# jac99/Egonn

Hardware: AMD Instinct MI355X
Metric: LiDAR scans/sec (descriptor extraction), 50k-pt clouds @ 0.1m voxel (higher is better)
Workload: dtype f32

## Files before the change

egonn_amd/_lib.py:

```python
from __future__ import annotations

import ctypes as C
import os
from typing import List, Optional, Sequence

import numpy as np
import torch

_HERE = os.path.dirname(os.path.abspath(__file__))
LIB_PATH = os.path.join(_HERE, "lib", "libegonn_hip.so")

QUANT_CARTESIAN, QUANT_POLAR = 0, 1
FLAG_DISABLE_GLOBAL, FLAG_DISABLE_LOCAL, FLAG_IGNORE_KP_REGRESSOR, FLAG_BF16 = 1, 2, 4, 8
FLAG_POOL_SPOC, FLAG_POOL_MAC = 16, 32
MINKFPN_SPLIT_TOPDOWN = 1
MINKFPN_BLOCKS = {'BasicBlock': 0, 'ECABasicBlock': 1}
MINKFPN_POOLING = {None: 0, 'GeM': 1, 'MAC': 2, 'SPoC': 3}

_P = C.c_void_p
_SIGS = [
    ("egonn_ctx_create", C.c_int, [C.POINTER(_P), C.c_int, C.c_int]),
    ("egonn_ctx_destroy", None, [_P]),
    ("egonn_last_error", C.c_char_p, []),
    ("egonn_debug_set_naive_conv", C.c_int, [_P, C.c_int]),
    ("egonn_debug_set_ksplit", C.c_int, [_P, C.c_int, C.c_int, C.c_int, C.c_int, C.c_int]),
    ("egonn_debug_set_resident", C.c_int, [_P, C.c_int, C.c_int]),
    ("egonn_debug_keep_level_features", C.c_int, [_P, C.c_int]),
    ("egonn_debug_set_trace", C.c_int, [_P]),
    ("egonn_prepare_maps", C.c_int, [_P, C.c_int, _P]),
    ("egonn_debug_rowgroup_tables", C.c_int, [_P, C.c_int, C.c_int, _P, _P, C.c_int64, C.POINTER(C.c_int64), _P]),
    ("egonn_debug_rowgroup_perm", C.c_int, [_P, C.c_int, C.c_int, _P, C.c_int64, C.POINTER(C.c_int64), _P]),
    ("egonn_debug_radix_sort_scratch_bytes", C.c_int64, [C.c_int64, C.c_int]),
    ("egonn_debug_radix_sort", C.c_int, [_P, _P, _P, _P, C.c_int64, C.c_int, _P, _P, C.c_int, C.c_int, C.c_int,
                                         C.POINTER(C.c_int32), _P, C.c_int64, _P]),
    ("egonn_voxelize", C.c_int, [_P, _P, C.POINTER(C.c_int64), C.c_int, C.c_int, C.POINTER(C.c_float), _P]),
    ("egonn_ctx_reserve", C.c_int, [_P, C.c_int64, C.c_int, C.POINTER(C.c_int64)]),
    ("egonn_voxelize_device", C.c_int, [_P, _P, C.c_int64, _P, C.c_int, C.c_int, C.POINTER(C.c_float), _P]),
    ("egonn_plan_status", C.c_int, [_P, _P]),
    ("egonn_ctx_set_exact_fp32", C.c_int, [_P, C.c_int]),
    ("egonn_ctx_set_operand_autoscale", C.c_int, [_P, C.c_int]),
    ("egonn_level_capacity", C.c_int, [_P, C.c_int, C.POINTER(C.c_int64)]),
    ("egonn_graph_begin", C.c_int, [_P]),
    ("egonn_graph_end", C.c_int, [_P, C.POINTER(_P)]),
    ("egonn_graph_launch", C.c_int, [_P, _P]),
    ("egonn_graph_destroy", None, [_P]),
    ("egonn_coords_set", C.c_int, [_P, _P, C.c_int64, C.c_int, _P]),
    ("egonn_level_count", C.c_int, [_P, C.c_int, C.POINTER(C.c_int64)]),
    ("egonn_level_batch_offsets", C.c_int, [_P, C.c_int, C.POINTER(C.c_int64)]),
    ("egonn_level_coords", C.c_int, [_P, C.c_int, _P, _P]),
    ("egonn_input_index", C.c_int, [_P, _P, _P]),
    ("egonn_conv", C.c_int, [_P, C.c_int, C.c_int, C.c_int, _P, C.c_int, _P, C.c_int, _P, _P, C.c_int, _P, _P]),
    ("egonn_conv_transpose", C.c_int, [_P, C.c_int, _P, C.c_int, _P, C.c_int, _P, _P]),
    ("egonn_sparse_conv", C.c_int, [_P, C.c_int, C.c_int, _P, C.c_int, _P, C.c_int, C.c_int, _P, _P, C.c_int, _P, _P, _P]),
    ("egonn_map_groups", C.c_int, [_P, C.c_int, C.c_int, C.POINTER(C.c_int64), C.POINTER(C.c_int64), _P]),
    ("egonn_global_avg_pool", C.c_int, [_P, C.c_int, _P, C.c_int, _P, _P]),
    ("egonn_bn_fold", C.c_int, [_P, _P, _P, _P, C.c_float, C.c_int, _P, _P, _P]),
    ("egonn_block_tail", C.c_int, [_P, C.c_int, _P, _P, C.c_int, _P, C.c_int, _P, _P]),
    ("egonn_gem", C.c_int, [_P, C.c_int, _P, C.c_int, _P, _P, _P]),
    ("egonn_global_max_pool", C.c_int, [_P, C.c_int, _P, C.c_int, _P, _P]),
    ("egonn_netvlad", C.c_int, [_P, C.c_int, _P, C.c_int, _P, _P, _P, _P, _P, _P, _P, _P, _P, _P, C.c_int, C.c_int, _P, _P]),
    ("egonn_netvlad_train_forward", C.c_int, [_P, C.c_int, _P, C.c_int, C.c_int, _P, _P, _P, _P, C.c_float, C.c_float, _P, _P,
                                              _P, C.c_int, _P, _P, _P, _P, _P, _P, _P]),
    ("egonn_netvlad_train_backward", C.c_int, [_P, C.c_int, _P, C.c_int, C.c_int, _P, _P, _P, _P, C.c_int, _P, _P, _P, _P, _P,
                                               _P, _P, _P, _P, _P, _P, _P]),
    ("egonn_global_max_pool_argmax", C.c_int, [_P, C.c_int, _P, C.c_int, _P, _P, _P]),
    ("egonn_global_max_pool_backward", C.c_int, [_P, C.c_int, _P, _P, C.c_int, _P, _P]),
    ("egonn_sigmoid_gate", C.c_int, [_P, _P, _P, C.c_int64, _P, _P, _P, _P]),
    ("egonn_add", C.c_int, [_P, _P, C.c_int64, _P, _P]),
    ("egonn_gather_input", C.c_int, [_P, _P, C.c_int, _P, _P]),
    ("egonn_model_create", C.c_int, [C.POINTER(_P)]),
    ("egonn_model_destroy", None, [_P]),
    ("egonn_model_set_tensor", C.c_int, [_P, C.c_char_p, _P, C.c_int, C.POINTER(C.c_int64)]),
    ("egonn_model_finalize", C.c_int, [_P, _P]),
    ("egonn_forward", C.c_int, [_P, _P, _P, C.c_int, C.POINTER(C.c_float), C.c_int, _P, _P, _P, _P, _P]),
    ("egonn_forward_level_features", C.c_int, [_P, C.c_int, _P, C.c_int, _P]),
    ("egonn_minkfpn_finalize", C.c_int, [_P, C.c_int, C.POINTER(C.c_int), C.POINTER(C.c_int), C.c_int, C.c_int, C.c_int, C.c_int, _P]),
    ("egonn_minkfpn_out_level", C.c_int, [C.c_int, C.c_int, C.POINTER(C.c_int)]),
    ("egonn_minkfpn_forward", C.c_int, [_P, _P, C.c_int, _P, _P, _P]),
    ("egonn_topdown_step", C.c_int, [_P, C.c_int, _P, _P, _P, _P, C.c_int, C.c_int, _P, _P]),
    ("egonn_select_keypoints", C.c_int, [_P, _P, _P, _P, C.c_int, _P, _P, _P, _P, _P]),
    ("egonn_topk_rows", C.c_int, [_P, _P, C.c_int, C.c_int, _P, _P, _P]),
    ("egonn_triplet_loss_scratch_floats", C.c_int64, [C.c_int]),
    ("egonn_triplet_loss", C.c_int, [_P, C.c_int, C.c_int, _P, _P, C.c_float, _P, _P, _P, _P, _P]),
    ("egonn_nn_search", C.c_int, [_P, C.c_int64, _P, _P, C.c_int64, _P, _P, _P]),
    ("egonn_matrix_min", C.c_int, [_P, C.c_int64, C.c_int64, _P, _P, _P, _P, _P]),
    ("egonn_softmax_cross_entropy", C.c_int, [_P, C.c_int64, C.c_int64, _P, _P, _P, _P, _P]),
    ("egonn_local_loss_scratch_bytes", C.c_int64, [C.c_int, C.c_int64, C.c_int64, C.c_int]),
    ("egonn_local_loss", C.c_int, [C.c_int, C.c_int64, C.c_int64, C.c_int64, C.c_int64, C.c_int] + [_P] * 13 +
                                  [C.POINTER(C.c_float)] + [_P] * 9 + [C.c_int64, _P]),
    ("egonn_dense", C.c_int, [_P, C.c_int64, C.c_int, _P, C.c_int, _P, C.c_int, C.c_int, _P, _P]),
    ("egonn_dense_pack_fragments", C.c_int, [_P, C.c_int, C.c_int, C.c_int, _P, _P]),
    ("egonn_dense_pack_fragments_host", C.c_int, [_P, C.c_int, C.c_int, C.c_int, _P]),
    ("egonn_debug_dense", C.c_int, [_P, C.c_int, C.c_int64, _P, C.c_int, C.c_int, _P, C.c_int, _P, _P, _P, _P, C.c_int, _P, C.c_int,
                                    _P, _P, C.c_int, _P, C.c_int, C.c_int, _P]),
    ("egonn_debug_dense_route", C.c_int, [C.c_int64, C.c_int, C.c_int, C.c_int, C.c_int, C.POINTER(C.c_int32)]),
    ("egonn_dense_backward_weight", C.c_int, [_P, C.c_int, _P, C.c_int, C.c_int64, _P, _P, C.c_int64, _P]),
    ("egonn_conv_backward_weight", C.c_int, [_P, C.c_int, C.c_int, C.c_int, C.c_int, _P, C.c_int, _P, C.c_int, _P, _P,
                                             C.c_int64, _P]),
    ("egonn_col_stats", C.c_int, [C.c_int, _P, _P, _P, _P, C.c_int64, C.c_int, _P, _P, C.c_int64, _P]),
    ("egonn_bn_train_finalize", C.c_int, [_P, _P, C.c_double, C.c_int, _P, _P, C.c_float, C.c_float, _P, _P, _P, _P]),
    ("egonn_bn_backward_finalize", C.c_int, [_P, _P, C.c_double, C.c_int, _P, _P, _P, _P, _P]),
    ("egonn_affine_act", C.c_int, [_P, _P, _P, C.c_int64, C.c_int, C.c_int, _P, _P]),
    ("egonn_affine3", C.c_int, [_P, _P, _P, _P, _P, _P, C.c_int64, C.c_int, _P, _P]),
    ("egonn_relu_backward", C.c_int, [_P, _P, C.c_int64, C.c_int, _P, _P]),
    ("egonn_contrastive_loss_scratch_floats", C.c_int64, [C.c_int]),
    ("egonn_contrastive_loss", C.c_int, [_P, C.c_int, C.c_int, _P, _P, C.c_float, C.c_float, _P, _P, _P, _P, _P]),
    ("egonn_se_gate", C.c_int, [_P, _P, _P, _P, _P, C.c_int, C.c_int, C.c_int, _P, _P, _P]),
    ("egonn_se_gate_backward", C.c_int, [_P, _P, _P, _P, _P, _P, C.c_int, C.c_int, C.c_int, _P, _P, _P, _P, _P, _P]),
    ("egonn_eca_gate", C.c_int, [_P, _P, C.c_int, C.c_int, C.c_int, _P, _P]),
    ("egonn_eca_gate_backward", C.c_int, [_P, _P, _P, _P, C.c_int, C.c_int, C.c_int, _P, _P, _P]),
    ("egonn_act_backward", C.c_int, [C.c_int, _P, _P, C.c_int64, C.c_int, _P, _P]),
    ("egonn_l2_normalize", C.c_int, [_P, _P, C.c_int64, C.c_int, _P, _P]),
    ("egonn_gate_residual", C.c_int, [_P, C.c_int, _P, _P, _P, C.c_int, C.c_int, _P, _P]),
    ("egonn_gate_residual_backward", C.c_int, [_P, C.c_int, _P, _P, _P, C.c_int, _P, _P, _P]),
    ("egonn_segment_sums", C.c_int, [_P, C.c_int, C.c_int, _P, _P, _P, _P, C.c_int, _P, _P, C.c_int64, _P]),
    ("egonn_segment_broadcast", C.c_int, [_P, C.c_int, _P, C.c_int, C.c_int, _P, _P]),
    ("egonn_gem_backward", C.c_int, [_P, C.c_int, _P, _P, _P, C.c_int, _P, _P]),
    ("egonn_filter_points_scratch_ints", C.c_int64, [C.c_int64]),
    ("egonn_filter_points", C.c_int, [_P, C.c_int64, C.c_int, _P, C.c_int, C.c_int, C.c_int, C.c_float, _P, _P, _P,
                                      C.c_int64, _P]),
    ("egonn_knn", C.c_int, [_P, C.c_int64, _P, C.c_int64, C.c_int, C.c_int, _P, _P, _P, C.c_int64, _P]),
    ("egonn_recall_counts", C.c_int, [_P, _P, _P, C.c_int64, C.c_int, C.c_int, _P, C.c_int, _P, _P]),
    ("egonn_registration_scratch_bytes", C.c_int64, [C.c_int, C.c_int, C.c_int]),
    ("egonn_match_mutual_scratch_bytes", C.c_int64, [C.c_int, C.c_int]),
    ("egonn_match_mutual", C.c_int, [_P, _P, _P, _P, C.c_int, C.c_int, C.c_int, _P, _P, _P, C.c_int64, _P]),
    ("egonn_ransac_pairs", C.c_int, [_P, _P, _P, _P, _P, _P, _P, C.c_int, C.c_int, C.c_int, C.c_uint64, C.c_double, _P,
                                     C.c_int64, _P, _P, _P]),
    ("egonn_registration_finish", C.c_int, [_P, _P, _P, _P, _P, _P, _P, C.c_int, C.c_int, C.c_int, C.c_uint64, C.c_double, _P,
                                            C.c_int64, _P, C.c_double, _P, _P, _P, _P, _P, _P, _P, _P, _P, _P, _P, _P]),
    ("egonn_voxel_downsample_scratch_bytes", C.c_int64, [C.c_int64, C.c_int]),
    ("egonn_voxel_downsample", C.c_int, [_P, C.c_int64, _P, C.c_int, C.c_double, C.POINTER(C.c_float), _P, _P, _P, _P, _P,
                                         C.c_int64, _P]),
    ("egonn_icp_scratch_bytes", C.c_int64, [C.c_int64, C.c_int64, C.c_int]),
    ("egonn_icp_pairs", C.c_int, [_P, C.c_int64, _P, _P, C.c_int64, _P, C.c_int, _P, C.c_double, C.c_int, C.c_double, C.c_double,
                                  _P, _P, _P, _P, _P, _P, _P, _P, _P, C.c_int64, _P]),
    ("egonn_estimate_normals_scratch_bytes", C.c_int64, [C.c_int64, C.c_int]),
    ("egonn_estimate_normals", C.c_int, [_P, C.c_int64, _P, C.c_int, C.c_int, _P, _P, _P, _P, _P, C.c_int64, _P]),
    ("egonn_icp_plane_scratch_bytes", C.c_int64, [C.c_int64, C.c_int64, C.c_int]),
    ("egonn_icp_plane_pairs", C.c_int, [_P, C.c_int64, _P, _P, C.c_int64, _P, _P, C.c_int, _P, C.c_double, C.c_int, C.c_double,
                                        C.c_double, _P, _P, _P, _P, _P, _P, _P, _P, _P, C.c_int64, _P]),
    ("egonn_augment_scratch_bytes", C.c_int64, [C.c_int64, C.c_int]),
    ("egonn_augment_points", C.c_int, [_P, C.c_int64, _P, C.c_int, _P, _P, _P, _P, _P, _P, _P, _P, _P, C.c_int64, _P]),
    ("egonn_scan_context", C.c_int, [_P, C.c_int64, _P, C.c_int, C.c_int, C.c_int, C.c_double, C.c_double, _P, _P, _P]),
    ("egonn_scan_context_ringkey", C.c_int, [_P, C.c_int64, C.c_int, C.c_int, _P, _P]),
    ("egonn_scan_context_distance", C.c_int, [_P, C.c_int64, _P, C.c_int64, C.c_int, C.c_int, _P, C.c_int, _P, _P, _P]),
    ("egonn_scan_context_rerank", C.c_int, [_P, _P, _P, C.c_int64, C.c_int, _P, _P, _P, _P]),
    ("egonn_radius_count", C.c_int, [_P, C.c_int64, _P, C.c_int64, C.POINTER(C.c_double), C.c_int, C.c_int, _P, _P]),
    ("egonn_radius_fill", C.c_int, [_P, C.c_int64, _P, C.c_int64, C.c_double, C.c_int, _P, _P, C.c_int64, _P, _P]),
    ("egonn_pair_masks", C.c_int, [_P, C.c_int, _P, _P, C.c_int64, _P, _P, C.c_int64, C.c_int64, _P, _P, _P, _P]),
    ("egonn_relative_poses", C.c_int, [_P, C.c_int64, _P, _P, C.c_int64, C.c_int, _P, _P, _P]),
    ("egonn_gather_clouds", C.c_int, [_P, C.c_int64, _P, C.c_int64, _P, C.c_int, _P, C.c_int64, _P, _P, _P]),
    ("egonn_match_candidates_scratch_bytes", C.c_int64, [C.c_int, C.c_int, C.c_int]),
    ("egonn_match_candidates", C.c_int, [_P, _P, _P, _P, _P, C.c_int, C.c_int, C.c_int, C.c_int, C.c_int, _P, _P, _P, _P,
                                         C.c_int64, _P]),
    ("egonn_gather_candidates", C.c_int, [_P, _P, _P, _P, _P, _P, C.c_int, C.c_int, C.c_int, C.c_int, _P, _P, _P, _P, _P, _P]),
    ("egonn_pick_candidates", C.c_int, [_P, C.c_int, C.c_int, C.c_int, _P, _P, _P, _P, _P, _P, _P, _P, C.c_int] + [_P] * 12),
    ("egonn_profile_enable", C.c_int, [_P, C.c_int, C.c_char_p]),
    ("egonn_profile_fetch", C.c_int, [_P, C.c_int, C.POINTER(C.c_int), C.c_char_p, C.POINTER(C.c_float),
                                      C.POINTER(C.c_double), C.POINTER(C.c_double), _P]),
]
EXPORTED_SYMBOLS = [s[0] for s in _SIGS]

_lib = None


def load() -> C.CDLL:
    global _lib
    if _lib is not None:
        return _lib
    if not os.path.exists(LIB_PATH):
        raise RuntimeError(
            f"egonn_amd: HIP library not found at {LIB_PATH}. Build it with "
            f"`python -c 'import __graft_entry__ as g; g.build()'` (hipcc --offload-arch=gfx950). "
            f"There is no CPU fallback.")
    lib = C.CDLL(LIB_PATH)
    for name, res, args in _SIGS:
        fn = getattr(lib, name)
        fn.restype = res
        fn.argtypes = args
    _lib = lib
    return lib


def _err(lib) -> str:
    msg = lib.egonn_last_error()
    return msg.decode() if msg else "unknown error"


class EgonnError(RuntimeError):

    def __init__(self, msg: str, code: int):
        super().__init__(msg)
        self.code = int(code)


class CapacityError(EgonnError):
    """status 5: the batch did not fit the capacities of egonn_ctx_reserve (the exact-size eager path still works)"""


class Fp16RangeError(EgonnError):
    """status 6: a kernel on the fp16-split pipe (fp32 sparse convolution or local heads) met an operand fp16 cannot hold
    (|x| >= 65520) or a non-finite input: the batch's outputs are invalid; Context.set_exact_fp32(True) and run it again
    (on the same plan: every forward clears this flag)"""


def check(rc: int):
    if rc != 0:
        cls = CapacityError if rc == 5 else (Fp16RangeError if rc == 6 else EgonnError)
        raise cls(f"libegonn_hip: {_err(load())} (code {rc})", rc)


def _stream() -> int:
    return torch.cuda.current_stream().cuda_stream


def _ptr(t: Optional[torch.Tensor]) -> Optional[int]:
    return None if t is None else t.data_ptr()


def call(device: torch.device, fn, *args):
    idx = device.index
    if idx is None or torch.cuda.current_device() == idx:
        rc = fn(*args, _stream())
    else:
        with torch.cuda.device(device):
            rc = fn(*args, _stream())
    if rc != 0:
        check(rc)


def _dev_f32(t: torch.Tensor, device) -> torch.Tensor:
    return t.to(device=device, dtype=torch.float32).contiguous()


def as_dev(x, dev, dtype) -> torch.Tensor:
    return torch.as_tensor(x).to(device=dev, dtype=dtype).contiguous()


def scratch(nbytes: int, dev) -> torch.Tensor:
    return torch.empty((max(int(nbytes), 8) + 7) // 8, dtype=torch.int64, device=dev)


def check_cloud(name, x):
    shape = tuple(getattr(x, "shape", ()))
    if len(shape) != 2 or shape[1] != 3:
        raise ValueError(f"{name}: expected (n, 3) points, got shape {shape}")


def check_offsets(name, off) -> int:
    shape = tuple(getattr(off, "shape", (len(off),) if hasattr(off, "__len__") else ()))
    if len(shape) != 1 or shape[0] < 2:
        raise ValueError(f"{name}: offsets must be a 1-D sequence of n_clouds + 1 entries, got shape {shape}")
    return shape[0] - 1


def concat_clouds(clouds, dev):
    ts = [torch.as_tensor(c) for c in clouds]
    for c in ts:
        check_cloud("cloud", c)
    off = [0]
    for c in ts:
        off.append(off[-1] + c.shape[0])
    pts = torch.cat([c.to(device=dev, dtype=torch.float32) for c in ts]) if ts else torch.zeros((0, 3), device=dev)
    return pts, torch.tensor(off, dtype=torch.int64, device=dev)


def dense_pack_fragments(weight, out_in: bool):
    lib = load()
    co, ci = (weight.shape if out_in else weight.shape[::-1])
    if isinstance(weight, np.ndarray):
        w = np.ascontiguousarray(weight, dtype=np.float32)
        out = np.empty(ci * co, dtype=np.float32)
        check(lib.egonn_dense_pack_fragments_host(w.ctypes.data, int(bool(out_in)), int(ci), int(co), out.ctypes.data))
        return out
    w = weight.contiguous()
    out = torch.empty(ci * co, dtype=torch.float32, device=w.device)
    call(w.device, lib.egonn_dense_pack_fragments, w.data_ptr(), int(bool(out_in)), int(ci), int(co), out.data_ptr())
    return out


def debug_dense(x, weight, out_in: bool, out, form: int, n_dev=None, packed=None, bias=None, scale=None, shift=None, act: int = 0,
                residual=None, gate=None, boff=None):
    lib = load()
    cap, cin = x.shape
    cout = out.shape[1]
    B = 0 if boff is None else boff.numel() - 1
    bf = lambda t: int(t is not None and t.dtype == torch.bfloat16)
    call(x.device, lib.egonn_debug_dense, x.data_ptr(), bf(x), int(cap), _ptr(n_dev), int(cin), int(cout), weight.data_ptr(),
         int(bool(out_in)), _ptr(packed), _ptr(bias), _ptr(scale), _ptr(shift), int(act), _ptr(residual), bf(residual), _ptr(gate),
         _ptr(boff), B, out.data_ptr(), bf(out), int(form))
    return out


DENSE_ROUTES = ("none", "stream", "lds", "small", "tile", "plain")


def debug_dense_route(rows: int, cin: int, cout: int, form: int = -1, gate_scans: int = 0):
    out = (C.c_int32 * 5)()
    check(load().egonn_debug_dense_route(int(rows), int(cin), int(cout), int(form), int(gate_scans), out))
    return (DENSE_ROUTES[out[0]],) + tuple(out[1:])


def debug_radix_sort(keys_in, vals_in, keys_out, vals_out, n: int, nbits: int, n_dev=None, seg_offsets=None, idx_bits: int = 0,
                     either_pair: bool = False, scratch_buf=None, scratch_bytes: Optional[int] = None) -> int:
    lib = load()
    B = 0 if seg_offsets is None else seg_offsets.numel() - 1
    need = lib.egonn_debug_radix_sort_scratch_bytes(int(n), B)
    if scratch_buf is None:
        scratch_buf = scratch(need, keys_in.device)
    pair = C.c_int32(-1)
    call(keys_in.device, lib.egonn_debug_radix_sort, keys_in.data_ptr(), vals_in.data_ptr(), keys_out.data_ptr(),
         vals_out.data_ptr(), int(n), int(nbits), _ptr(n_dev), _ptr(seg_offsets), B, int(idx_bits), int(bool(either_pair)),
         C.byref(pair), scratch_buf.data_ptr(), need if scratch_bytes is None else int(scratch_bytes))
    return pair.value


def require_gpu() -> torch.device:
    if not torch.cuda.is_available():
        raise RuntimeError("egonn_amd: no HIP device visible (torch.cuda.is_available() is False); "
                           "the descriptor-extraction path runs on MI355X only — there is no CPU fallback.")
    return torch.device("cuda", torch.cuda.current_device())


class Context:

    def __init__(self, device: Optional[torch.device] = None, coord_bits: int = 16):
        self.lib = load()
        self.device = torch.device(device) if device is not None else require_gpu()
        if self.device.type != "cuda":
            raise RuntimeError(f"egonn_amd: device {self.device} is not a HIP device; there is no CPU fallback.")
        if self.device.index is None:
            self.device = torch.device("cuda", torch.cuda.current_device())
        h = _P()
        check(self.lib.egonn_ctx_create(C.byref(h), self.device.index, coord_bits))
        self.h = h
        self.batch_size = 0
        self._keep = []

    def __del__(self):
        try:
            if getattr(self, "h", None):
                self.lib.egonn_ctx_destroy(self.h)
                self.h = None
        except Exception:
            pass

    def voxelize(self, points: torch.Tensor, scan_offsets: Sequence[int], mode: int, step: Sequence[float]):
        assert points.is_cuda and points.dtype == torch.float32 and points.is_contiguous()
        assert points.dim() == 2 and points.shape[1] == 3
        B = len(scan_offsets) - 1
        off = (C.c_int64 * (B + 1))(*[int(o) for o in scan_offsets])
        st = (C.c_float * 3)(*([float(s) for s in step] + [0.0, 0.0])[:3])
        self._call(self.lib.egonn_voxelize, self.h, points.data_ptr(), off, B, mode, st)
        self.batch_size = B

    def reserve(self, max_points: int, batch_size: int, level_capacity: Optional[Sequence[int]] = None):
        caps = None
        if level_capacity is not None:
            assert len(level_capacity) == 8
            caps = (C.c_int64 * 8)(*[int(v) for v in level_capacity])
        with torch.cuda.device(self.device):
            check(self.lib.egonn_ctx_reserve(self.h, int(max_points), int(batch_size), caps))
        self.batch_size = int(batch_size)

    def voxelize_device(self, points: torch.Tensor, scan_offsets: torch.Tensor, batch_size: int, mode: int,
                        step: Sequence[float]):
        assert points.is_cuda and points.dtype == torch.float32 and points.is_contiguous() and points.shape[1] == 3
        assert scan_offsets.is_cuda and scan_offsets.dtype == torch.int64 and scan_offsets.numel() == batch_size + 1
        st = (C.c_float * 3)(*([float(s) for s in step] + [0.0, 0.0])[:3])
        self._call(self.lib.egonn_voxelize_device, self.h, points.data_ptr(), points.shape[0], scan_offsets.data_ptr(),
                   int(batch_size), mode, st)
        self.batch_size = int(batch_size)

    def plan_status(self):
        self._call(self.lib.egonn_plan_status, self.h)

    def level_capacity(self, level: int) -> int:
        n = C.c_int64()
        check(self.lib.egonn_level_capacity(self.h, level, C.byref(n)))
        return n.value

    def coords_set(self, coords: torch.Tensor, batch_size: int):
        assert coords.is_cuda and coords.dtype == torch.int32 and coords.is_contiguous()
        assert coords.dim() == 2 and coords.shape[1] == 4
        self._call(self.lib.egonn_coords_set, self.h, coords.data_ptr(), coords.shape[0], int(batch_size))
        self.batch_size = int(batch_size)

    def level_count(self, level: int) -> int:
        n = C.c_int64()
        check(self.lib.egonn_level_count(self.h, level, C.byref(n)))
        return n.value

    def level_batch_offsets(self, level: int) -> List[int]:
        off = (C.c_int64 * (self.batch_size + 1))()
        check(self.lib.egonn_level_batch_offsets(self.h, level, off))
        return list(off)

    def level_coords(self, level: int) -> torch.Tensor:
        out = torch.empty((self.level_count(level), 4), dtype=torch.int32, device=self.device)
        self._call(self.lib.egonn_level_coords, self.h, level, out.data_ptr())
        return out

    def input_index(self) -> torch.Tensor:
        out = torch.empty((self.level_count(0),), dtype=torch.int64, device=self.device)
        self._call(self.lib.egonn_input_index, self.h, out.data_ptr())
        return out

    def conv(self, level_in: int, level_out: int, kernel_size: int, x: torch.Tensor, kernel: torch.Tensor,
             scale: Optional[torch.Tensor] = None, shift: Optional[torch.Tensor] = None, relu: bool = False):
        kernel = _dev_f32(kernel, self.device)
        cin, cout = kernel.shape[-2], kernel.shape[-1]
        if x is None:
            assert kernel_size == 5 and cin == 1, "x=None (all-ones features) is the k=5 input layer only"
        else:
            x = _dev_f32(x, self.device)
            assert x.shape == (self.level_count(level_in), cin), (x.shape, self.level_count(level_in), cin)
        out = torch.empty((self.level_count(level_out), cout), dtype=torch.float32, device=self.device)
        sc = None if scale is None else _dev_f32(scale, self.device)
        sh = None if shift is None else _dev_f32(shift, self.device)
        self._call(self.lib.egonn_conv, self.h, level_in, level_out, kernel_size, _ptr(x), cin, kernel.data_ptr(), cout,
                   _ptr(sc), _ptr(sh), int(relu), out.data_ptr())
        return out

    def conv_transpose(self, level_in: int, x: torch.Tensor, kernel: torch.Tensor):
        x = _dev_f32(x, self.device)
        kernel = _dev_f32(kernel, self.device)
        cin, cout = kernel.shape[-2], kernel.shape[-1]
        assert x.shape == (self.level_count(level_in), cin)
        out = torch.empty((self.level_count(level_in - 1), cout), dtype=torch.float32, device=self.device)
        self._call(self.lib.egonn_conv_transpose, self.h, level_in, x.data_ptr(), cin, kernel.data_ptr(), cout, out.data_ptr())
        return out

    def sparse_conv(self, map_kind: int, level_out: int, x: torch.Tensor, kernel: torch.Tensor, scale=None, shift=None,
                    relu: bool = False, group_sums: bool = False):
        assert x.is_cuda and x.dtype in (torch.float32, torch.bfloat16) and x.is_contiguous()
        kernel = _dev_f32(kernel, self.device)
        cin, cout = kernel.shape[-2], kernel.shape[-1]
        assert x.shape[1] == cin
        out = torch.empty((self.level_count(level_out), cout), dtype=x.dtype, device=self.device)
        sc = None if scale is None else _dev_f32(scale, self.device)
        sh = None if shift is None else _dev_f32(shift, self.device)
        sums = None
        if group_sums:
            sums = torch.zeros((self.map_groups(map_kind, level_out)[0], cout), dtype=torch.float32, device=self.device)
        self._call(self.lib.egonn_sparse_conv, self.h, map_kind, level_out, x.data_ptr(), cin, kernel.data_ptr(), cout,
                   int(x.dtype == torch.bfloat16), _ptr(sc), _ptr(sh), int(relu), out.data_ptr(), _ptr(sums))
        return (out, sums) if group_sums else out

    def prepare_maps(self, with_level0_transpose: bool = False):
        self._call(self.lib.egonn_prepare_maps, self.h, int(with_level0_transpose))

    def map_groups(self, map_kind: int, level_out: int):
        n = C.c_int64()
        first = (C.c_int64 * (self.batch_size + 1))()
        self._call(self.lib.egonn_map_groups, self.h, map_kind, level_out, C.byref(n), first)
        return n.value, list(first)

    def rowgroup_tables(self, map_kind: int, level_out: int, with_rows: bool = True):
        ng, _ = self.map_groups(map_kind, level_out)
        K = 27 if map_kind == 0 else 8
        gm = torch.empty(ng, dtype=torch.int32, device=self.device)
        sn = torch.empty((ng, K, 16), dtype=torch.int32, device=self.device) if with_rows else None
        n = C.c_int64()
        self._call(self.lib.egonn_debug_rowgroup_tables, self.h, map_kind, level_out, gm.data_ptr(),
                   sn.data_ptr() if with_rows else None, ng, C.byref(n))
        return gm, sn

    def rowgroup_perm(self, map_kind: int, level_out: int):
        ng, _ = self.map_groups(map_kind, level_out)
# ... 409 lines not shown
```

egonn_amd/csrc/common.h:

```cpp
#pragma once
#include <hip/hip_runtime.h>
#include <atomic>
#include <stdint.h>
#include <stdio.h>
#include <string.h>
#include <string>
#include <vector>

#define EGONN_MAX_LEVELS 10
#define EGONN_NUM_LEVELS 8
#define EGONN_MAX_BATCH 4096

#define API extern "C" __attribute__((visibility("default")))

namespace egonn {

void set_error(const char* fmt, ...);
#define EGONN_OK 0
#define EGONN_ERR_INVALID 1
#define EGONN_ERR_HIP 2
#define EGONN_ERR_RANGE 3
#define EGONN_ERR_STATE 4
#define EGONN_ERR_CAPACITY 5
#define EGONN_ERR_FP16_RANGE 6
// ... 26 lines not shown
__host__ __device__ static inline int clipi(int v, int hi) { return v < 0 ? 0 : (v > hi ? hi : v); }
__host__ __device__ static inline int64_t clipi(int64_t v, int64_t hi) { return v < 0 ? 0 : (v > hi ? hi : v); }

struct AttrOnce {
  std::atomic<uint64_t> done{0};
  static int dev() { int d = 0; (void)hipGetDevice(&d); return d & 63; }
  bool need() const { return !((done.load(std::memory_order_acquire) >> dev()) & 1ull); }
  void mark() { done.fetch_or(1ull << dev(), std::memory_order_release); }
};
static inline size_t align_up(size_t v, size_t a) { return (v + a - 1) / a * a; }

struct Arena {
  char* base = nullptr;
  size_t cap = 0;
  size_t off = 0;
  bool borrowed = false;
  static Arena view(void* span, size_t bytes) {
    Arena a;
    a.base = static_cast<char*>(span);
    a.cap = bytes;
    a.borrowed = true;
    return a;
  }
  int ensure(size_t bytes) {
    if (bytes <= cap) return EGONN_OK;
    EGONN_REQUIRE(!borrowed, EGONN_ERR_INVALID, "scratch span of %zu bytes is %zu bytes short of the %zu needed", cap, bytes - cap,
                  bytes);
    size_t want = align_up(bytes + bytes / 4, size_t(1) << 20);
    if (base) {
      HIP_CHECK(hipDeviceSynchronize());
      HIP_CHECK(hipFree(base));
      base = nullptr;
      cap = 0;
    }
    HIP_CHECK(hipMalloc(reinterpret_cast<void**>(&base), want));
    cap = want;
    off = 0;
    return EGONN_OK;
  }
  void reset() { off = 0; }
  template <typename T>
  T* alloc(size_t n) {
    size_t o = align_up(off, 256);
    size_t end = o + n * sizeof(T);
    if (end > cap) return nullptr;
    off = end;
    return reinterpret_cast<T*>(base + o);
  }
  void release() {
    if (borrowed) return;
    if (base) (void)hipFree(base);
    base = nullptr;
    cap = off = 0;
  }
};

__host__ __device__ static inline uint64_t part1by2(uint32_t v) {
  uint64_t x = v & 0xFFFFull;
  x = (x | (x << 16)) & 0x0000FF0000FFull;
  x = (x | (x << 8)) & 0x00F00F00F00Full;
  x = (x | (x << 4)) & 0x0C30C30C30C3ull;
  x = (x | (x << 2)) & 0x249249249249ull;
  return x;
}
__host__ __device__ static inline uint32_t compact1by2(uint64_t x) {
  x &= 0x249249249249ull;
  x = (x | (x >> 2)) & 0x0C30C30C30C3ull;
  x = (x | (x >> 4)) & 0x00F00F00F00Full;
  x = (x | (x >> 8)) & 0x0000FF0000FFull;
  x = (x | (x >> 16)) & 0xFFFFull;
  return (uint32_t)x;
}
__host__ __device__ static inline uint64_t morton3(uint32_t x, uint32_t y, uint32_t z) {
  return part1by2(x) | (part1by2(y) << 1) | (part1by2(z) << 2);
}

static constexpr int RG_MAX_JOBS = 24;
static constexpr int RG_MAX_WIN = 512;
struct RowGroups {
  int K = 0;
  int win = 0;
  int cap_groups = 0;
  int32_t* perm = nullptr;
  int32_t* snbr = nullptr;
  uint32_t* gmask = nullptr;
  int32_t* meta = nullptr;
  int32_t* order4 = nullptr;
  bool built = false;
};
struct RGBuild {
  RowGroups* rg;
  const int32_t* nbr;
  const int32_t* n_dev;
  const int32_t* boff;
  int32_t cap_rows = 0;
};
int rowgroup_build(const RGBuild* jobs, int njobs, int B, hipStream_t stream);

struct Level {
  int64_t n = 0;
  uint64_t* keys = nullptr;
  int32_t* parent = nullptr;
  int32_t* cstart = nullptr;
  uint64_t* mask = nullptr;
  int32_t* bstart = nullptr;
  int32_t* boff = nullptr;
  int32_t* nbr27 = nullptr;
  int32_t* nbr8 = nullptr;
  int32_t* nbrT = nullptr;
  RowGroups rg27, rg8, rgT;
};

struct Plan {
  bool valid = false;
  bool built_reserved = false;
  bool exact = false;
  int64_t cap_points = 0;
  int64_t* scan_off = nullptr;
  int batch = 0;
  int coord_bits = 16;
  int64_t n_input = 0;
  Level lv[EGONN_MAX_LEVELS];
  int64_t cap[EGONN_MAX_LEVELS] = {};
  int32_t* perm0 = nullptr;
  int32_t* g0 = nullptr;
  uint64_t* t2m = nullptr;
  int32_t* t2s = nullptr;
  std::vector<int32_t> boff_host[EGONN_NUM_LEVELS];
};

enum ProfKind { PK_CONV0 = 0, PK_K3 = 1, PK_K2S2 = 2, PK_TCONV = 3, PK_OTHER = 4 };
struct ProfRec {
  char name[64];
  int kind, level, K, cin, cout;
  int es;
  hipEvent_t e0, e1;
};
struct Profiler {
  int mode = 0;
  char filter[64] = "";
  std::vector<ProfRec> recs;
  std::vector<ProfRec> graph_recs;
  std::vector<hipEvent_t> pool;
  hipEvent_t get();
};

struct Switches {
  bool debug_sync;
  bool no_presplit;
  bool no_fused_down;
  bool no_fused_lateral;
  bool no_gated_k2s2;
  bool no_fused_ghead;
  bool no_split_heads;
  bool no_tail_split;
  bool no_task_order;
  bool flat_sort, sort_pairs;
  bool no_search67;
  bool no_dense_stream;
  int split_max_level;
  int split_max_level_k8;
  int split_cfg;
  int rg_first_pass;
  const char* ksplit[5];
};
const Switches& switches();

struct KsRule {
  int8_t kparts[2][EGONN_NUM_LEVELS];
  int8_t kw[2][EGONN_NUM_LEVELS];
  int8_t col_parts[EGONN_NUM_LEVELS];
};

static constexpr int SCONV_RESIDENT_DEFAULT = 6;

struct Ctx {
  Profiler prof;
  KsRule ks_rule;
  uint16_t* conv0_lut = nullptr;
  unsigned long long* dev_pairs = nullptr;
  int device = 0;
  int coord_bits = 16;
  int split_max_level = 5;
  float* ks_part = nullptr;
  size_t ks_part_floats = 0;
  const void* sort_prezeroed = nullptr;
  int resident_mask = SCONV_RESIDENT_DEFAULT;
  int resident_wgs = 0;
  int keep_level_features = 0;
  int operand_autoscale = 0;
  int conv_variant = 0;
  Arena plan_arena;
  Arena work_arena;
  Arena sort_arena;
  Plan plan;
  int32_t* host_counts = nullptr;
  int32_t* dev_counts = nullptr;
  int32_t* dev_flags = nullptr;
  int32_t* dev_fp16_flag = nullptr;
  bool reserved = false;
  int64_t reserve_points = 0;
  int reserve_batch = 0;
  int64_t reserve_cap[EGONN_MAX_LEVELS] = {};
  hipEvent_t ev0 = nullptr, ev1 = nullptr;
};

hipEvent_t* prof_kernel_events();
struct ProfScope {
  Ctx* ctx;
  hipStream_t st;
  int idx = -1;
  bool exact = false;
  bool in_graph = false;
  ProfScope(Ctx* c, hipStream_t s, const char* name, int kind, int level, int K, int cin, int cout, int es);
  ~ProfScope();
};

int ensure_level0_parent_table(Ctx* ctx, hipStream_t stream);
int ensure_rowgroups(Ctx* ctx, const int* kinds, const int* levels, int count, hipStream_t stream);
int rowgroup_cap_groups(const Plan& P, int level);

static constexpr int KP_MAX_N = 256;
static constexpr int KP_MAX_D = 256;
static constexpr int KP_MAX_PAIRS = 1 << 20;
static constexpr int REL_MAX_K = 1024;
int reg_check_shape(const char* who, int P, int n_max);
int rel_check_shape(const char* who, int Q, int k, int M, int n_max);

int radix_sort_pairs(Arena& ws, uint64_t* keys_in, uint32_t* vals_in, uint64_t* keys_out, uint32_t* vals_out,
                     int64_t n, int nbits, hipStream_t stream, const int64_t* n_dev = nullptr, uint64_t** keys_res = nullptr,
                     uint32_t** vals_res = nullptr);
size_t radix_sort_scratch_bytes(int64_t n);
int radix_sort_segments(Arena& ws, uint64_t* keys_in, uint32_t* vals_in, uint64_t* keys_out, uint32_t* vals_out, int64_t n,
                        const int64_t* off_dev, int B, int nbits, hipStream_t stream, uint64_t** keys_res, uint32_t** vals_res,
                        int idx_bits = 0, const void* prezeroed = nullptr);
size_t radix_sort_segments_scratch_bytes(int64_t n, int B);
int radix_sort_segments_layout(Arena& ws, int64_t n, int B, int32_t** tilehist, int32_t** scanhist);
int radix_sort_segments_passes(int nbits);
int radix_sort_segments_digits();

int plan_from_points(Ctx* ctx, const float* points, const int64_t* scan_offsets, int64_t n_cap, int offsets_on_device,
                     int B, int mode, const float* step, hipStream_t stream);
int plan_reserve(Ctx* ctx, int64_t max_points, int B, const int64_t* level_caps);
int plan_sync(Ctx* ctx, hipStream_t stream);
int plan_from_coords(Ctx* ctx, const int32_t* coords, int64_t n, int B, hipStream_t stream);
int plan_level_coords(Ctx* ctx, int level, int32_t* out, hipStream_t stream);
int count_map_pairs(Ctx* ctx, hipStream_t stream);

}
```

egonn_amd/csrc/coords.hip:

```cpp
#include "common.h"

#include <algorithm>
#include <stdarg.h>

namespace egonn {

static thread_local char g_err[1024] = "";
void set_error(const char* fmt, ...) {
  va_list ap;
  va_start(ap, fmt);
  vsnprintf(g_err, sizeof(g_err), fmt, ap);
  va_end(ap);
}
const char* last_error() { return g_err; }

const Switches& switches() {
  static const Switches sw = [] {
    auto on = [](const char* name) { return getenv(name) != nullptr; };
    auto num = [](const char* name, int unset) { const char* e = getenv(name); return e ? atoi(e) : unset; };
    const char* ds = getenv("EGONN_DEBUG_SYNC");
    return Switches{.debug_sync = ds && ds[0] == '1', .no_presplit = on("EGONN_NO_PRESPLIT"), .no_fused_down = on("EGONN_NO_FUSED_DOWN"),
                    .no_fused_lateral = on("EGONN_NO_FUSED_LATERAL"), .no_gated_k2s2 = on("EGONN_NO_GATED_K2S2"),
                    .no_fused_ghead = on("EGONN_NO_FUSED_GHEAD"), .no_split_heads = on("EGONN_NO_SPLIT_HEADS"),
                    .no_tail_split = on("EGONN_NO_TAIL_SPLIT"), .no_task_order = on("EGONN_NO_TASK_ORDER"),
                    .flat_sort = on("EGONN_FLAT_SORT"), .sort_pairs = on("EGONN_SORT_PAIRS"), .no_search67 = on("EGONN_NO_SEARCH67"),
                    .no_dense_stream = on("EGONN_NO_DENSE_STREAM"),
                    .split_max_level = num("EGONN_SPLIT_MAX_LEVEL", -1), .split_max_level_k8 = num("EGONN_SPLIT_MAX_LEVEL_K8", -1),
                    .split_cfg = num("EGONN_SPLIT_CFG", 0), .rg_first_pass = num("EGONN_RG_FIRST_PASS", 0),
                    .ksplit = {getenv("EGONN_KSPLIT"), getenv("EGONN_KSPLIT8"), getenv("EGONN_KSPLIT_KW"), getenv("EGONN_KSPLIT_KW8"),
                               getenv("EGONN_KSPLIT_PARTS")}};
  }();
  return sw;
}

hipEvent_t Profiler::get() {
  if (!pool.empty()) {
    hipEvent_t e = pool.back();
    pool.pop_back();
    return e;
  }
  hipEvent_t e = nullptr;
  (void)hipEventCreate(&e);
  return e;
}
ProfScope::ProfScope(Ctx* c, hipStream_t s, const char* name, int kind, int level, int K, int cin, int cout, int es)
    : ctx(c), st(s) {
  if (!c || c->prof.mode == 0) return;
  if (c->prof.mode >= 2 && !strstr(name, c->prof.filter)) return;
  hipStreamCaptureStatus cs = hipStreamCaptureStatusNone;
  (void)hipStreamIsCapturing(s, &cs);
  in_graph = cs == hipStreamCaptureStatusActive;
  if (in_graph && c->prof.mode != 3) return;
  ProfRec r;
  snprintf(r.name, sizeof(r.name), "%s", name);
  r.kind = kind; r.level = level; r.K = K; r.cin = cin; r.cout = cout; r.es = es;
  r.e0 = c->prof.get();
  r.e1 = c->prof.get();
  exact = c->prof.mode == 2 && (kind == PK_K3 || kind == PK_K2S2 || kind == PK_TCONV);
  if (exact) {
    prof_kernel_events()[0] = r.e0;
    prof_kernel_events()[1] = r.e1;
  } else {
    (void)hipEventRecord(r.e0, s);
  }
  std::vector<ProfRec>& dst = in_graph ? c->prof.graph_recs : c->prof.recs;
  idx = (int)dst.size();
  dst.push_back(r);
}
ProfScope::~ProfScope() {
  if (idx < 0) return;
  if (exact) {
    prof_kernel_events()[0] = prof_kernel_events()[1] = nullptr;
  } else {
    (void)hipEventRecord((in_graph ? ctx->prof.graph_recs : ctx->prof.recs)[idx].e1, st);
  }
}
hipEvent_t* prof_kernel_events() {
  static thread_local hipEvent_t ev[2] = {nullptr, nullptr};
  return ev;
}

struct QuantParams {
  int mode;
  float s0, s1, s2;
};

__device__ static inline void quantize_point(const QuantParams& qp, float x, float y, float z, int32_t& cx,
                                             int32_t& cy, int32_t& cz) {
  if (qp.mode == 0) {
    cx = (int32_t)floorf(qp.s0 == 1.0f ? x : __fdiv_rn(x, qp.s0));
    cy = (int32_t)floorf(qp.s0 == 1.0f ? y : __fdiv_rn(y, qp.s0));
    cz = (int32_t)floorf(qp.s0 == 1.0f ? z : __fdiv_rn(z, qp.s0));
  } else {
    const float at = (float)atan2((double)y, (double)x);
    const float theta = __fadd_rn(180.0f, __fdiv_rn(__fmul_rn(at, 180.0f), 3.14159265358979323846f));
    const float dist = sqrtf(__fadd_rn(__fmul_rn(x, x), __fmul_rn(y, y)));
    cx = (int32_t)floorf(__fdiv_rn(theta, qp.s0));
    cy = (int32_t)floorf(__fdiv_rn(dist, qp.s1));
    cz = (int32_t)floorf(__fdiv_rn(z, qp.s2));
  }
}

__device__ static inline bool encode_key(int32_t b, int32_t cx, int32_t cy, int32_t cz, int cb, uint64_t& key) {
  const int32_t bias = 1 << (cb - 1);
  const int32_t lim = 1 << cb;
  const int32_t ux = cx + bias, uy = cy + bias, uz = cz + bias;
  const bool ok = (ux >= 0) & (ux < lim) & (uy >= 0) & (uy < lim) & (uz >= 0) & (uz < lim) & (b >= 0);
  key = ((uint64_t)(uint32_t)b << (3 * cb)) | morton3((uint32_t)ux, (uint32_t)uy, (uint32_t)uz);
  return ok;
}

__global__ void points_to_keys_kernel(const float* __restrict__ pts, int64_t n_cap, const int64_t* __restrict__ scan_off,
                                      int B, QuantParams qp, int cb, uint64_t* __restrict__ keys,
                                      uint32_t* __restrict__ vals, int32_t* __restrict__ flags, int idx_bits,
                                      int64_t* __restrict__ off_copy, int32_t* __restrict__ zero_ptr, int zero_words) {
  const int64_t i = (int64_t)blockIdx.x * blockDim.x + threadIdx.x;
  const int64_t stride = (int64_t)gridDim.x * blockDim.x;
  if (off_copy)
    for (int64_t b = i; b <= B; b += stride) off_copy[b] = scan_off[b];
  for (int64_t w = i; w < zero_words; w += stride) zero_ptr[w] = 0;
  const int64_t nn = scan_off[B];
  if (i == 0 && nn > n_cap) atomicOr(flags, 2);
  for (int64_t b = i; b <= B; b += stride)
    if ((b == 0 && scan_off[0] != 0) || (b > 0 && scan_off[b] < scan_off[b - 1])) atomicOr(flags, 1);
  if (i >= (nn < n_cap ? nn : n_cap)) return;
  int lo = 0, hi = B;
  while (hi - lo > 1) {
    const int mid = (lo + hi) >> 1;
    if (scan_off[mid] <= i) lo = mid; else hi = mid;
  }
  const float x = pts[3 * i + 0], y = pts[3 * i + 1], z = pts[3 * i + 2];
  int32_t cx, cy, cz;
  quantize_point(qp, x, y, z, cx, cy, cz);
  uint64_t key;
  const bool finite = isfinite(x) & isfinite(y) & isfinite(z);
  if (!encode_key(lo, cx, cy, cz, cb, key) || !finite) {
    atomicOr(flags, 1);
    const int32_t hi = (1 << (cb - 1)) - 1, lo_c = -(1 << (cb - 1));
    const int32_t qx = finite ? min(max(cx, lo_c), hi) : 0, qy = finite ? min(max(cy, lo_c), hi) : 0,
                  qz = finite ? min(max(cz, lo_c), hi) : 0;
    encode_key(lo, qx, qy, qz, cb, key);
  }
  if (idx_bits > 0) {
    keys[i] = ((key & ((1ull << (3 * cb)) - 1)) << idx_bits) | (uint64_t)(i - scan_off[lo]);
  } else {
    keys[i] = key;
    vals[i] = (uint32_t)i;
  }
}

__global__ void coords_to_keys_kernel(const int32_t* __restrict__ c4, int64_t n, int cb, int Bmax,
                                      uint64_t* __restrict__ keys, uint32_t* __restrict__ vals,
                                      int32_t* __restrict__ flags) {
  const int64_t i = (int64_t)blockIdx.x * blockDim.x + threadIdx.x;
  if (i >= n) return;
  const int4 c = reinterpret_cast<const int4*>(c4)[i];
  uint64_t key;
  if (!encode_key(c.x, c.y, c.z, c.w, cb, key) || c.x >= Bmax) {
    atomicOr(flags, 1);
    key = ~0ull >> 1;
  }
  keys[i] = key;
  vals[i] = (uint32_t)i;
}

static constexpr int PYR_BLOCK = 256;
static constexpr int PYR_ROUNDS = 4;
static constexpr int PYR_TILE = PYR_BLOCK * PYR_ROUNDS;
static constexpr int NL = EGONN_MAX_LEVELS;

__device__ static inline int head_levels(const uint64_t* __restrict__ keys, int64_t i) {
  if (i == 0) return NL;
  const uint64_t d = keys[i] ^ keys[i - 1];
  if (d == 0) return 0;
  const int t = (63 - __clzll(d)) / 3;
  return (t >= NL - 1) ? NL : t + 1;
// ... 902 lines not shown
```

egonn_amd/csrc/dense.hip:

```cpp
#include <algorithm>
#include <type_traits>

#include "../../include/egonn_hip.h"
#include "common.h"
#include "kernels.h"
#include "rowmath.h"

namespace egonn {

template <int W_OUT_IN, int CIN, bool IN_BF16>
__global__ __launch_bounds__(256) void dense_kernel(const void* __restrict__ in_v, int64_t n,
                                                    const float* __restrict__ W, int cout,
                                                    const float* __restrict__ bias, const float* __restrict__ scale,
                                                    const float* __restrict__ shift, int act,
                                                    const void* __restrict__ residual_v, void* __restrict__ out_v, int io,
                                                    const int32_t* __restrict__ n_dev) {
  if (n_dev) n = min((int64_t)*n_dev, n);
  const float* in = reinterpret_cast<const float*>(in_v);
  const float* residual = reinterpret_cast<const float*>(residual_v);
  float* out = reinterpret_cast<float*>(out_v);
  constexpr int KS = CIN / 16;
  const int lane = threadIdx.x & 63, wave = threadIdx.x >> 6;
  const int l15 = lane & 15, g4 = lane >> 4;
  const int64_t row_base = ((int64_t)blockIdx.x * 4 + wave) * 16;
  if (row_base >= n) return;
  const int64_t row = row_base + l15;
  float4 a[KS];
#pragma unroll
  for (int t = 0; t < KS; ++t) {
    a[t] = make_float4(0, 0, 0, 0);
    if (row < n) {
      if constexpr (IN_BF16) {
        const uint2 h = *reinterpret_cast<const uint2*>(reinterpret_cast<const uint16_t*>(in_v) + row * CIN + 16 * t + 4 * g4);
        a[t] = make_float4(bf2f(h.x & 0xFFFFu), bf2f(h.x >> 16), bf2f(h.y & 0xFFFFu), bf2f(h.y >> 16));
      } else {
        a[t] = *reinterpret_cast<const float4*>(in + row * CIN + 16 * t + 4 * g4);
      }
    }
  }
  const int ncol0 = blockIdx.y * 64;
#pragma unroll 1
  for (int pass = 0; pass < 2; ++pass) {
    const int n0 = ncol0 + pass * 32;
    if (n0 >= cout) break;
    float4 b[2][KS];
#pragma unroll
    for (int nt = 0; nt < 2; ++nt) {
      const int col = n0 + nt * 16 + l15;
#pragma unroll
      for (int t = 0; t < KS; ++t) {
        float4 v = make_float4(0, 0, 0, 0);
        if (col < cout) {
          if (W_OUT_IN) {
            v = *reinterpret_cast<const float4*>(W + (int64_t)col * CIN + 16 * t + 4 * g4);
          } else {
            const float* wp = W + (int64_t)(16 * t + 4 * g4) * cout + col;
            v.x = wp[0];
            v.y = wp[cout];
            v.z = wp[2 * (int64_t)cout];
            v.w = wp[3 * (int64_t)cout];
          }
        }
        b[nt][t] = v;
      }
    }
    f32x4 acc[2] = {{0.f, 0.f, 0.f, 0.f}, {0.f, 0.f, 0.f, 0.f}};
#pragma unroll
    for (int t = 0; t < KS; ++t) {
#pragma unroll
      for (int nt = 0; nt < 2; ++nt) {
        acc[nt] = __builtin_amdgcn_mfma_f32_16x16x4f32(a[t].x, b[nt][t].x, acc[nt], 0, 0, 0);
        acc[nt] = __builtin_amdgcn_mfma_f32_16x16x4f32(a[t].y, b[nt][t].y, acc[nt], 0, 0, 0);
        acc[nt] = __builtin_amdgcn_mfma_f32_16x16x4f32(a[t].z, b[nt][t].z, acc[nt], 0, 0, 0);
        acc[nt] = __builtin_amdgcn_mfma_f32_16x16x4f32(a[t].w, b[nt][t].w, acc[nt], 0, 0, 0);
      }
    }
#pragma unroll
    for (int nt = 0; nt < 2; ++nt) {
      const int col = n0 + nt * 16 + l15;
      if (col < cout) {
        const float bi = bias ? bias[col] : 0.f;
        const float sc = scale ? scale[col] : 1.f, sh = scale ? shift[col] : 0.f;
#pragma unroll
        for (int r = 0; r < 4; ++r) {
          const int64_t orow = row_base + 4 * g4 + r;
          if (orow < n) {
            float v = acc[nt][r] + bi;
            if (scale) v = v * sc + sh;
            v = apply_act(v, act);
            if (residual_v)
              v += (io & 1) ? bf2f(reinterpret_cast<const uint16_t*>(residual_v)[orow * cout + col]) : residual[orow * cout + col];
            if (io & 2) reinterpret_cast<uint16_t*>(out_v)[orow * cout + col] = (uint16_t)f2bf_rn(v);
            else out[orow * cout + col] = v;
          }
        }
      }
    }
  }
}

template <int W_OUT_IN, int CIN, bool IN_BF16>
__device__ static inline void dense_small_body(const void* __restrict__ in_v, int64_t n,
                                               const float* __restrict__ W, int cout,
                                               const float* __restrict__ bias, const float* __restrict__ scale,
                                               const float* __restrict__ shift, int act,
                                               const void* __restrict__ residual_v, void* __restrict__ out_v, int io,
                                               const int32_t* __restrict__ n_dev, const int block_x, const int block_y) {
  const int64_t ncap = n;
  const int32_t* nd = n_dev ? n_dev : reinterpret_cast<const int32_t*>(W);
  const int32_t nlive_raw = *nd;
  const int32_t nlive32 = n_dev ? nlive_raw : 0x7FFFFFFF;
  const float* in = reinterpret_cast<const float*>(in_v);
  float* out = reinterpret_cast<float*>(out_v);
  constexpr int KS = CIN / 16;
  const int lane = threadIdx.x & 63, wave = threadIdx.x >> 6;
  const int l15 = lane & 15, g4 = lane >> 4;
  const int64_t row_base = ((int64_t)block_x * 4 + wave) * 16;
  if (row_base >= ncap) return;
  const int64_t row = min(row_base + l15, ncap - 1);
  float4 a[KS];
#pragma unroll
  for (int t = 0; t < KS; ++t) {
    if constexpr (IN_BF16) {
      const uint2 h = *reinterpret_cast<const uint2*>(reinterpret_cast<const uint16_t*>(in_v) + row * CIN + 16 * t + 4 * g4);
      a[t] = make_float4(bf2f(h.x & 0xFFFFu), bf2f(h.x >> 16), bf2f(h.y & 0xFFFFu), bf2f(h.y >> 16));
    } else {
      a[t] = *reinterpret_cast<const float4*>(in + row * CIN + 16 * t + 4 * g4);
    }
  }
  const int ncol0 = block_y * 64;
  float4 b[4][KS];
  float bi[4], sc[4], sh[4];
  const float* bias_p = bias ? bias : W;
  const float* scale_p = scale ? scale : W;
  const float* shift_p = scale ? shift : W;
#pragma unroll
  for (int nt = 0; nt < 4; ++nt) {
    const int col = min(ncol0 + nt * 16 + l15, cout - 1);
    bi[nt] = bias_p[col];
    sc[nt] = scale_p[col];
    sh[nt] = shift_p[col];
#pragma unroll
    for (int t = 0; t < KS; ++t) {
      float4 v;
      if (W_OUT_IN) {
        v = *reinterpret_cast<const float4*>(W + (int64_t)col * CIN + 16 * t + 4 * g4);
      } else {
        const float* wp = W + (int64_t)(16 * t + 4 * g4) * cout + col;
        v.x = wp[0];
        v.y = wp[cout];
        v.z = wp[2 * (int64_t)cout];
        v.w = wp[3 * (int64_t)cout];
      }
      b[nt][t] = v;
    }
  }
  float res[4][4];
  {
    const bool has_res = residual_v != nullptr;
    const void* rp = has_res ? residual_v : static_cast<const void*>(W);
    int64_t ridx[4][4];
#pragma unroll
    for (int nt = 0; nt < 4; ++nt) {
      const int col = min(ncol0 + nt * 16 + l15, cout - 1);
#pragma unroll
      for (int r = 0; r < 4; ++r) {
        const int64_t orow = min(row_base + 4 * g4 + r, ncap - 1);
        ridx[nt][r] = has_res ? orow * cout + col : 0;
      }
    }
    if (io & 1) {
#pragma unroll
      for (int nt = 0; nt < 4; ++nt)
#pragma unroll
        for (int r = 0; r < 4; ++r) res[nt][r] = bf2f(reinterpret_cast<const uint16_t*>(rp)[ridx[nt][r]]);
    } else {
#pragma unroll
      for (int nt = 0; nt < 4; ++nt)
#pragma unroll
        for (int r = 0; r < 4; ++r) res[nt][r] = reinterpret_cast<const float*>(rp)[ridx[nt][r]];
    }
  }
  if (!bias) bi[0] = bi[1] = bi[2] = bi[3] = 0.f;
  n = min((int64_t)nlive32, ncap);
  if (row_base >= n) return;
#pragma unroll
  for (int nt = 0; nt < 4; ++nt) {
    const int col = ncol0 + nt * 16 + l15;
    if (ncol0 + nt * 16 >= cout) break;
    f32x4 acc = {0.f, 0.f, 0.f, 0.f};
#pragma unroll
    for (int t = 0; t < KS; ++t) {
      acc = __builtin_amdgcn_mfma_f32_16x16x4f32(a[t].x, b[nt][t].x, acc, 0, 0, 0);
      acc = __builtin_amdgcn_mfma_f32_16x16x4f32(a[t].y, b[nt][t].y, acc, 0, 0, 0);
      acc = __builtin_amdgcn_mfma_f32_16x16x4f32(a[t].z, b[nt][t].z, acc, 0, 0, 0);
      acc = __builtin_amdgcn_mfma_f32_16x16x4f32(a[t].w, b[nt][t].w, acc, 0, 0, 0);
    }
    if (col < cout) {
#pragma unroll
      for (int r = 0; r < 4; ++r) {
        const int64_t orow = row_base + 4 * g4 + r;
        if (orow < n) {
          float v = acc[r] + bi[nt];
          if (scale) v = v * sc[nt] + sh[nt];
          v = apply_act(v, act);
          if (residual_v) v += res[nt][r];
          if (io & 2) reinterpret_cast<uint16_t*>(out_v)[orow * cout + col] = (uint16_t)f2bf_rn(v);
          else out[orow * cout + col] = v;
        }
      }
    }
  }
}

template <int W_OUT_IN, int CIN, bool IN_BF16>
__global__ __launch_bounds__(256) void dense_small_kernel(const void* __restrict__ in_v, int64_t n,
                                                    const float* __restrict__ W, int cout,
                                                    const float* __restrict__ bias, const float* __restrict__ scale,
                                                    const float* __restrict__ shift, int act,
                                                    const void* __restrict__ residual_v, void* __restrict__ out_v, int io,
                                                    const int32_t* __restrict__ n_dev) {
  dense_small_body<W_OUT_IN, CIN, IN_BF16>(in_v, n, W, cout, bias, scale, shift, act, residual_v, out_v, io, n_dev, (int)blockIdx.x,
                                           (int)blockIdx.y);
}
struct DenseGroup3 {
  const void* in[3];
  const float* W[3];
  void* out[3];
  const int32_t* n_dev[3];
  int64_t n[3];
  int bx0[4];
};
template <int W_OUT_IN, int CIN, bool IN_BF16>
__global__ __launch_bounds__(256) void dense_small3_kernel(const DenseGroup3 g, int cout, int io) {
  const int b = (int)blockIdx.x;
  const int q = b >= g.bx0[2] ? 2 : (b >= g.bx0[1] ? 1 : 0);
  dense_small_body<W_OUT_IN, CIN, IN_BF16>(g.in[q], g.n[q], g.W[q], cout, nullptr, nullptr, nullptr, ACT_NONE, nullptr, g.out[q], io,
                                           g.n_dev[q], b - g.bx0[q], (int)blockIdx.y);
}


template <int W_OUT_IN, int CIN, bool IN_BF16>
__global__ __launch_bounds__(256) void dense_lds_kernel(const void* __restrict__ in_v, int64_t n,
                                                        const float* __restrict__ W, int cout,
                                                        const float* __restrict__ bias, const float* __restrict__ scale,
                                                        const float* __restrict__ shift, int act,
                                                        const void* __restrict__ residual_v, void* __restrict__ out_v, int io,
                                                        const int32_t* __restrict__ n_dev, int colblk,
                                                        const float* __restrict__ gate, const int32_t* __restrict__ boff, int B) {
  extern __shared__ __attribute__((aligned(16))) f32x4 dl_frags[];
  if (n_dev) n = min((int64_t)*n_dev, n);
  constexpr int KS = CIN / 16;
  const int tid = threadIdx.x, lane = tid & 63, wave = tid >> 6;
  const int l15 = lane & 15, g4 = lane >> 4;
  const int cb0 = blockIdx.y * colblk;
  const int NT = min(colblk, cout - cb0) >> 4, ncl = NT * 16;
  auto frag_of = [&](int i) -> f32x4 {
    const int ln = i & 63, ft = i >> 6;
    const int nt = ft / KS, t = ft - nt * KS;
    const int col = cb0 + 16 * nt + (ln & 15), k0 = 16 * t + 4 * (ln >> 4);
    if (W_OUT_IN) return *reinterpret_cast<const f32x4*>(W + (int64_t)col * CIN + k0);
    const float* wp = W + (int64_t)k0 * cout + col;
    return (f32x4){wp[0], wp[cout], wp[2 * (int64_t)cout], wp[3 * (int64_t)cout]};
  };
  const int nfrag = NT * KS * 64;
  int i0 = tid;
  for (; i0 + 7 * 256 < nfrag; i0 += 8 * 256) {
    f32x4 v[8];
#pragma unroll
    for (int u = 0; u < 8; ++u) v[u] = frag_of(i0 + u * 256);
#pragma unroll
    for (int u = 0; u < 8; ++u) dl_frags[i0 + u * 256] = v[u];
  }
  for (; i0 < nfrag; i0 += 256) dl_frags[i0] = frag_of(i0);
  __syncthreads();
  float* const s_vec = reinterpret_cast<float*>(dl_frags + (int64_t)NT * KS * 64);
  for (int i = tid; i < ncl; i += 256) {
    s_vec[i] = bias ? bias[cb0 + i] : 0.f;
    s_vec[ncl + i] = scale ? scale[cb0 + i] : 1.f;
    s_vec[2 * ncl + i] = scale ? shift[cb0 + i] : 0.f;
  }
  __syncthreads();
  const int64_t ntiles = (n + 15) >> 4;
  const int64_t tstep = (int64_t)gridDim.x * 4;
  auto load_rows = [&](int64_t tile, f32x4 (&a)[KS]) {
    const int64_t row = tile * 16 + l15;
#pragma unroll
    for (int t = 0; t < KS; ++t) {
      a[t] = (f32x4){0.f, 0.f, 0.f, 0.f};
      if (tile < ntiles && row < n) {
        if constexpr (IN_BF16) {
          const uint2 h = *reinterpret_cast<const uint2*>(reinterpret_cast<const uint16_t*>(in_v) + row * CIN + 16 * t + 4 * g4);
          a[t] = (f32x4){bf2f(h.x & 0xFFFFu), bf2f(h.x >> 16), bf2f(h.y & 0xFFFFu), bf2f(h.y >> 16)};
        } else {
          a[t] = *reinterpret_cast<const f32x4*>(reinterpret_cast<const float*>(in_v) + row * CIN + 16 * t + 4 * g4);
        }
      }
    }
  };
  f32x4 a[KS], an[KS];
  int64_t tile = (int64_t)blockIdx.x * 4 + wave;
  load_rows(tile, a);
  for (; tile < ntiles; tile += tstep) {
    const int64_t row = tile * 16 + l15;
    const bool ok = row < n;
    load_rows(tile + tstep, an);
    const int64_t gbase = (gate && ok) ? (int64_t)sample_of_row(boff, B, (int32_t)row) * cout : 0;
    for (int nt = 0; nt < NT; ++nt) {
      f32x4 acc = {0.f, 0.f, 0.f, 0.f};
      const f32x4* fr = dl_frags + (int64_t)nt * KS * 64 + lane;
#pragma unroll
      for (int t = 0; t < KS; ++t) {
        const f32x4 wf = fr[t * 64];
#pragma unroll
        for (int u = 0; u < 4; ++u) acc = __builtin_amdgcn_mfma_f32_16x16x4f32(wf[u], a[t][u], acc, 0, 0, 0);
      }
      if (ok) {
        const int cl = 16 * nt + 4 * g4, c0 = cb0 + cl;
        f32x4 v = acc + *reinterpret_cast<const f32x4*>(s_vec + cl);
        v = v * *reinterpret_cast<const f32x4*>(s_vec + ncl + cl) + *reinterpret_cast<const f32x4*>(s_vec + 2 * ncl + cl);
#pragma unroll
        for (int u = 0; u < 4; ++u) v[u] = apply_act(v[u], act);
        if (residual_v) {
          f32x4 r;
          if (io & 1) {
            const uint2 h = *reinterpret_cast<const uint2*>(reinterpret_cast<const uint16_t*>(residual_v) + row * cout + c0);
            r = (f32x4){bf2f(h.x & 0xFFFFu), bf2f(h.x >> 16), bf2f(h.y & 0xFFFFu), bf2f(h.y >> 16)};
          } else {
            r = *reinterpret_cast<const f32x4*>(reinterpret_cast<const float*>(residual_v) + row * cout + c0);
          }
          if (gate) {
            const f32x4 gq = *reinterpret_cast<const f32x4*>(gate + gbase + c0);
#pragma unroll
            for (int u = 0; u < 4; ++u) {
              const float d = (io & 2) ? bf2f(f2bf_rn(v[u])) : v[u];
              v[u] = fmaxf(r[u] * gq[u] + d, 0.f);
            }
          } else {
            v += r;
          }
        }
        if (io & 2) {
// ... 137 lines not shown
#pragma unroll
      for (int u = 0; u < 4; ++u) v[u] = ACT_ANY ? apply_act(v[u], act) : (act == ACT_RELU ? fmaxf(v[u], 0.f) : v[u]);
      if (residual_v) {
        f32x4 rr = r[nt];
        if (io & 1) {
          const uint32_t hx = __float_as_uint(rr[0]), hy = __float_as_uint(rr[1]);
          rr = (f32x4){bf2f(hx & 0xFFFFu), bf2f(hx >> 16), bf2f(hy & 0xFFFFu), bf2f(hy >> 16)};
        }
        if (gate) {
#pragma unroll
          for (int u = 0; u < 4; ++u) {
            const float d = (io & 2) ? bf2f(f2bf_rn(v[u])) : v[u];
            v[u] = fmaxf(rr[u] * gq[nt][u] + d, 0.f);
          }
        } else {
          v += rr;
        }
      }
      if (io & 2) {
        *reinterpret_cast<uint2*>(reinterpret_cast<uint16_t*>(out_v) + row * COUT + c0) =
            make_uint2(f2bf_rn(v[0]) | (f2bf_rn(v[1]) << 16), f2bf_rn(v[2]) | (f2bf_rn(v[3]) << 16));
      } else {
        *reinterpret_cast<f32x4*>(reinterpret_cast<float*>(out_v) + row * COUT + c0) = v;
      }
    }
    __builtin_amdgcn_sched_barrier(0);
  }
}

__global__ void dense_any_kernel(const float* __restrict__ in, int64_t total, int cin, const float* __restrict__ W,
                                 int w_out_in, int cout, const float* __restrict__ bias, int act, float* __restrict__ out,
                                 const int32_t* __restrict__ n_dev) {
  const int64_t i = (int64_t)blockIdx.x * blockDim.x + threadIdx.x;
  if (n_dev) total = min((int64_t)*n_dev * cout, total);
  if (i >= total) return;
  const int64_t r = i / cout;
  const int co = (int)(i - r * cout);
  float s = bias ? bias[co] : 0.f;
  for (int ci = 0; ci < cin; ++ci) s = fmaf(in[r * cin + ci], w_out_in ? W[(int64_t)co * cin + ci] : W[(int64_t)ci * cout + co], s);
  out[i] = apply_act(s, act);
}

constexpr int64_t DENSE_STAGED_ROWS = 8192;
constexpr int64_t DENSE_STAGED_ROWS_SPLIT = 2048;
constexpr size_t DENSE_STREAM_MAX_BYTES = 32 * 1024;
constexpr size_t DENSE_LDS_BLOCK_BYTES = 96 * 1024;
constexpr size_t DENSE_LDS_TWO_WG_BYTES = 72 * 1024;
constexpr int DENSE_LDS_WGS[2] = {512, 256};
constexpr int DENSE_SMALL_MAX_CIN = 128;

template <int... V, class F>
static bool pick(int v, F&& f) { return ((v == V && (f(std::integral_constant<int, V>{}), true)) || ...); }
template <class F>
static bool pick_cin(int cin, F&& f) { return pick<32, 64, 96, 128, 192, 256>(cin, f); }
template <class F>
static void dense_dispatch(const DenseCall& c, F&& f) {
  pick_cin(c.cin, [&](auto CI) { pick<0, 1>(c.w_out_in != 0, [&](auto WOI) { pick<0, 1>(c.in_bf16 != 0, [&](auto INB) {
    f(CI, WOI, std::bool_constant<INB != 0>{}); }); }); });
}
constexpr bool dense_stream_plan(int cin, int cout) {
  return (cin == 32 || cin == 64 || cin == 128) && (cout == 64 || cout == 128) && (size_t)cin * cout * sizeof(float) <= DENSE_STREAM_MAX_BYTES;
}

DenseLaunch dense_launch(int64_t n, int cin, int cout, int form, int gate_scans) {
  DenseLaunch l;
  if (n == 0) return l;
  const size_t wbytes = (size_t)cin * cout * sizeof(float);
  const unsigned wave_tiles = (unsigned)cdiv(cdiv(n, 16), 4);
  const bool stream_shape = n >= DENSE_STAGED_ROWS && dense_stream_plan(cin, cout);
  const int ysplit = (int)cdiv((int64_t)wbytes, DENSE_LDS_BLOCK_BYTES);
  if (form == 1 && !stream_shape) {
    l.route = DENSE_INVALID;
  } else if (form == 1 || (form < 0 && !switches().no_dense_stream && stream_shape)) {
    l = {DENSE_STREAM, wave_tiles, 1, wbytes + 3 * cout * sizeof(float) + ((size_t)gate_scans + 1) * sizeof(int32_t)};
  } else if (!pick_cin(cin, [](auto) {})) {
    l = {DENSE_PLAIN, (unsigned)cdiv(n * cout, 256), 1};
  } else if (cout % 16 == 0 && n >= (ysplit == 1 ? DENSE_STAGED_ROWS : DENSE_STAGED_ROWS_SPLIT)) {
    const int colblk = (int)(cdiv(cdiv(cout, ysplit), 16) * 16);
    const size_t blk_bytes = (size_t)cin * colblk * sizeof(float);
    const unsigned ny = (unsigned)cdiv(cout, colblk);
    l = {DENSE_LDS, std::min(wave_tiles, DENSE_LDS_WGS[blk_bytes > DENSE_LDS_TWO_WG_BYTES] / ny), ny, blk_bytes + 3 * colblk * sizeof(float), colblk};
  } else {
    l = {n < DENSE_STAGED_ROWS && cin <= DENSE_SMALL_MAX_CIN ? DENSE_SMALL : DENSE_TILE, (unsigned)cdiv(n, 64), (unsigned)cdiv(cout, 64)};
  }
  return l;
}
DenseRoute dense_route(int64_t n, int cin, int cout, int form) { return dense_launch(n, cin, cout, form, 0).route; }
bool dense_gate_fusable(int64_t n, int cin, int cout) {
  const DenseLaunch l = dense_launch(n, cin, cout, 0, 0);
  return l.route == DENSE_LDS && l.gy == 1;
}
static int dense_plan(int64_t n, int cin, int cout, int form, bool gate, int B, DenseLaunch* l) {
  EGONN_REQUIRE(!gate || (B >= 1 && dense_gate_fusable(n, cin, cout)), EGONN_ERR_INVALID,
                "dense: the fused gated residual needs the LDS-staged kernel (%lld rows, %d->%d)", (long long)n, cin, cout);
  *l = dense_launch(n, cin, cout, form, gate ? B : 0);
  EGONN_REQUIRE(l->route != DENSE_INVALID, EGONN_ERR_INVALID, "dense: no streaming form for %lld rows, %d->%d", (long long)n, cin, cout);
  return EGONN_OK;
}
template <int WOI, int CI, bool INB>
static int dense_lds_launch(const DenseCall& c, const DenseLaunch& l, int io, hipStream_t stream) {
  static AttrOnce attr_done;
  if (attr_done.need()) {
    HIP_CHECK(hipFuncSetAttribute(reinterpret_cast<const void*>(&dense_lds_kernel<WOI, CI, INB>), hipFuncAttributeMaxDynamicSharedMemorySize,
                                  160 * 1024));
    attr_done.mark();
  }
  hipLaunchKernelGGL((dense_lds_kernel<WOI, CI, INB>), dim3(l.gx, l.gy), dim3(256), l.lds, stream, c.in, c.n, c.W, c.cout, c.bias, c.scale,
                     c.shift, c.act, c.residual, c.out, io, c.n_dev, l.colblk, c.gate, c.boff, c.B);
  return EGONN_OK;
}

int dense_forward(const DenseCall& c, hipStream_t stream) {
  if (c.n == 0) return EGONN_OK;
  DenseLaunch l;
  EGONN_TRY(dense_plan(c.n, c.cin, c.cout, c.form, c.gate != nullptr, (c.residual && c.boff) ? c.B : 0, &l));
  const dim3 grid(l.gx, l.gy), block(256);
  const int io = (c.res_bf16 ? 1 : 0) | (c.out_bf16 ? 2 : 0);
  int rc = EGONN_OK;
  switch (l.route) {
    case DENSE_STREAM:
      pick_cin(c.cin, [&](auto CI) { pick<64, 128>(c.cout, [&](auto CO) { pick<0, 1>(c.in_bf16 != 0, [&](auto INB) {
        pick<0, 1>(c.act != ACT_NONE && c.act != ACT_RELU, [&](auto ANY) {
          if constexpr (dense_stream_plan(CI, CO))
            hipLaunchKernelGGL((dense_stream_kernel<CI, CO, INB != 0, ANY != 0>), grid, block, l.lds, stream, c.in, c.n, c.W, c.w_out_in,
                               c.wfrag, c.bias, c.scale, c.shift, c.act, c.residual, c.out, io, c.n_dev, c.gate, c.boff, c.B);
        }); }); }); });
      break;
    case DENSE_LDS:
      dense_dispatch(c, [&](auto CI, auto WOI, auto INB) { rc = dense_lds_launch<WOI, CI, INB>(c, l, io, stream); });
      break;
    case DENSE_SMALL:
    case DENSE_TILE:
      dense_dispatch(c, [&](auto CI, auto WOI, auto INB) {
        auto kernel = &dense_kernel<WOI, CI, INB>;
        if constexpr (CI <= DENSE_SMALL_MAX_CIN)
          if (l.route == DENSE_SMALL) kernel = &dense_small_kernel<WOI, CI, INB>;
        hipLaunchKernelGGL(kernel, grid, block, 0, stream, c.in, c.n, c.W, c.cout, c.bias, c.scale, c.shift, c.act, c.residual, c.out, io, c.n_dev);
      });
      break;
    case DENSE_PLAIN:
      EGONN_REQUIRE(!c.scale && !c.shift && !c.residual && !c.in_bf16 && !c.out_bf16, EGONN_ERR_INVALID, "dense: cin=%d has no fused epilogue",
                    c.cin);
      hipLaunchKernelGGL(dense_any_kernel, grid, block, 0, stream, reinterpret_cast<const float*>(c.in), c.n * c.cout, c.cin, c.W, c.w_out_in,
                         c.cout, c.bias, c.act, reinterpret_cast<float*>(c.out), c.n_dev);
      break;
    default: break;
  }
  EGONN_TRY(rc);
  HIP_CHECK(hipGetLastError());
  return EGONN_OK;
}

bool dense_group3_rows(int64_t n) { return n == 0 || dense_route(n, 128, 128, -1) == DENSE_SMALL; }
int dense_small_group3(const float* const* in, const int64_t* n, const int32_t* const* n_dev, const float* const* W, float* const* out,
                       hipStream_t stream) {
  DenseGroup3 g;
  int bx = 0;
  for (int q = 0; q < 3; ++q) {
    EGONN_REQUIRE(dense_group3_rows(n[q]), EGONN_ERR_INVALID, "dense(group): %lld rows", (long long)n[q]);
    g.in[q] = in[q]; g.W[q] = W[q]; g.out[q] = out[q]; g.n_dev[q] = n_dev[q]; g.n[q] = n[q];
    g.bx0[q] = bx;
    bx += (int)cdiv(std::max<int64_t>(n[q], 1), 64);
  }
  g.bx0[3] = bx;
  hipLaunchKernelGGL((dense_small3_kernel<0, 128, false>), dim3((unsigned)bx, 2), dim3(256), 0, stream, g, 128, 0);
  HIP_CHECK(hipGetLastError());
  return EGONN_OK;
}

}

using namespace egonn;

API int egonn_dense(const float* x, int64_t n, int cin, const float* weight, int weight_out_in, const float* bias, int cout,
                    int act, float* out, void* stream) {
  EGONN_REQUIRE(x && weight && out && n >= 0 && cin >= 1 && cout >= 1 && act >= 0 && act <= 4, EGONN_ERR_INVALID,
                "dense: bad arguments");
  return dense_forward({.in = x, .n = n, .cin = cin, .cout = cout, .W = weight, .w_out_in = weight_out_in ? 1 : 0, .bias = bias, .act = act,
                        .out = out},
                       (hipStream_t)stream);
}
API int egonn_dense_pack_fragments(const float* weight, int weight_out_in, int cin, int cout, float* packed, void* stream) {
  return dense_pack_frags(weight, weight_out_in, cin, cout, packed, (hipStream_t)stream);
}
API int egonn_dense_pack_fragments_host(const float* weight, int weight_out_in, int cin, int cout, float* packed) {
  EGONN_REQUIRE(weight && packed && cin >= 16 && cin % 16 == 0 && cout >= 16 && cout % 16 == 0, EGONN_ERR_INVALID,
                "dense pack: %d->%d (multiples of 16 expected)", cin, cout);
  for (int64_t j = 0; j < (int64_t)cin * cout; ++j) packed[j] = weight[dense_frag_src(j, weight_out_in ? 1 : 0, cin, cout)];
  return EGONN_OK;
}
API int egonn_debug_dense(const void* in, int in_bf16, int64_t rows_capacity, const int32_t* n_dev, int cin, int cout, const float* weight,
                          int weight_out_in, const float* packed, const float* bias, const float* scale, const float* shift, int act,
                          const void* residual, int res_bf16, const float* gate, const int32_t* boff, int B, void* out, int out_bf16,
                          int form, void* stream) {
  EGONN_REQUIRE(in && weight && out && rows_capacity >= 0 && cin >= 1 && cout >= 1 && act >= 0 && act <= 4 && (form == 0 || form == 1) &&
                    (!scale == !shift) && (form == 1 || !packed),
                EGONN_ERR_INVALID, "debug_dense: bad arguments");
  return dense_forward({.in = in, .in_bf16 = in_bf16 ? 1 : 0, .n = rows_capacity, .n_dev = n_dev, .cin = cin, .cout = cout, .W = weight,
                        .w_out_in = weight_out_in ? 1 : 0, .wfrag = packed, .bias = bias, .scale = scale, .shift = shift, .act = act,
                        .residual = residual, .res_bf16 = res_bf16 ? 1 : 0, .gate = gate, .boff = boff, .B = B, .out = out,
                        .out_bf16 = out_bf16 ? 1 : 0, .form = form},
                       (hipStream_t)stream);
}
API int egonn_debug_dense_route(int64_t rows, int cin, int cout, int form, int gate_scans, int32_t out[5]) {
  EGONN_REQUIRE(out && rows >= 0 && cin >= 1 && cout >= 1 && form >= -1 && form <= 1 && gate_scans >= 0, EGONN_ERR_INVALID,
                "debug_dense_route: bad arguments");
  DenseLaunch l;
  if (rows > 0) EGONN_TRY(dense_plan(rows, cin, cout, form, gate_scans > 0, gate_scans, &l));
  out[0] = l.route; out[1] = (int32_t)l.gx; out[2] = (int32_t)l.gy; out[3] = (int32_t)l.lds; out[4] = l.colblk;
  return EGONN_OK;
}
```

egonn_amd/csrc/kernels.h:

```cpp
#pragma once
#include "common.h"

namespace egonn {

const char* last_error();

bool sconv_rg_supported(int cin, int cout);
int pack_rg_weights(const float* W, int K, int cin, int cout, int bf16, int flip, int transpose, void* out,
                    hipStream_t stream);
extern unsigned long long* g_sconv_trace;
struct PackedKernel {
  const void* rg32 = nullptr;
  const void* rg16 = nullptr;
  const void* split = nullptr;
};
struct ConvCall {
  int kind = 0, level = 0;
  const void* in = nullptr; void* out = nullptr;
  int cin = 0, cout = 0, bf16 = 0;
  const float *scale = nullptr, *shift = nullptr;
  int relu = 0;
  float* psum = nullptr;
  const PackedKernel* packed = nullptr;
  const float* W = nullptr; float* scratch = nullptr; size_t scratch_floats = 0;
  int split_io = 0;
  const float *in2 = nullptr, *gate = nullptr;
  const float* residual = nullptr;
};
enum SconvRoute {
  ROUTE_PLAIN,
  ROUTE_SPLIT,
  ROUTE_TAIL_SPLIT,
  ROUTE_WG,
  ROUTE_DMA,
  ROUTE_RG
};
SconvRoute sconv_route(const Ctx* ctx, int kind, int level, int cin, int cout, int bf16);
bool sconv_split_arithmetic(const Ctx* ctx);
const char* sconv_kernel_name(const Ctx* ctx, int kind, int level, int cin, int cout, int bf16);
struct SconvLaunch {
  SconvRoute route = ROUTE_RG;
  const RowGroups* rg = nullptr;
  int64_t n_in_cap = 0;
  int64_t groups_hint = 0;
  const void* Wp = nullptr;
  int variant = 0;
  bool small = false;
  int32_t* flags = nullptr;
  int B = 0;
  int kparts = 1, kw = 0, col_parts = 0;
  int resident = 0, resident_wgs = 0;
  float* part = nullptr; size_t part_floats = 0;
  uint32_t* in_absmax = nullptr; int64_t in_elems = 0;
};
int sconv_rg_forward(const ConvCall& c, const SconvLaunch& l, hipStream_t stream);
int sconv_map(Ctx* ctx, const ConvCall& c, hipStream_t stream);
bool sconv_split_supported(int cin, int cout);
int pack_split_weights(const float* W, int K, int cin, int cout, int flip, int transpose, void* out, hipStream_t stream);
size_t split_weights_bytes(int K, int cin, int cout);
int sconv_split_forward(const ConvCall& c, const SconvLaunch& l, hipStream_t stream);
size_t sconv_split_part_floats(const RowGroups& rg, int cout, int kparts);
void sconv_ksplit_rule(const Ctx* ctx, int kind, int level, int* kparts, int* col_parts, int* kw);
void sconv_ksplit_defaults(KsRule* r);
size_t sconv_ksplit_scratch_floats(const Ctx* ctx);
int sconv_resident_bit(int kind, int level, int cin, int cout, bool gated);
static constexpr size_t SCONV_SCRATCH_FLOATS = (size_t)2 << 20;
int sconv_naive(const float* in, const int32_t* nbr, const float* W, const float* scale, const float* shift, int relu,
                float* out, int64_t n_out, int K, int cin, int cout, hipStream_t stream);
int conv0_lut_init(Ctx* ctx);
int conv0_k5_forward(Ctx* ctx, const float* feat, const float* W, int cout, const float* scale,
                     const float* shift, int relu, void* out, int out_bf16, hipStream_t stream, const void* wpk = nullptr);
int conv0_pack_unit(const float* W, void* wpk, hipStream_t stream);

enum Act { ACT_NONE = 0, ACT_RELU = 1, ACT_TANH = 2, ACT_SOFTPLUS = 3, ACT_SIGMOID = 4 };
struct DenseCall {
  const void* in = nullptr; int in_bf16 = 0;
  int64_t n = 0;
  const int32_t* n_dev = nullptr;
  int cin = 0, cout = 0;
  const float* W = nullptr;
  int w_out_in = 0;
  const float* wfrag = nullptr;
  const float* bias = nullptr;
  const float *scale = nullptr, *shift = nullptr;
  int act = 0;
  const void* residual = nullptr; int res_bf16 = 0;
  const float* gate = nullptr;
  const int32_t* boff = nullptr;
  int B = 0;
  void* out = nullptr; int out_bf16 = 0;
  int form = -1;
};
enum DenseRoute {
  DENSE_INVALID = -1,
  DENSE_NONE = 0,
  DENSE_STREAM,
  DENSE_LDS,
  DENSE_SMALL,
  DENSE_TILE,
  DENSE_PLAIN
};
struct DenseLaunch {
  DenseRoute route = DENSE_NONE;
  unsigned gx = 0, gy = 0;
  size_t lds = 0;
  int colblk = 0;
};
DenseRoute dense_route(int64_t n, int cin, int cout, int form);
DenseLaunch dense_launch(int64_t n, int cin, int cout, int form, int gate_scans);
int dense_forward(const DenseCall& c, hipStream_t stream);
bool dense_gate_fusable(int64_t n, int cin, int cout);
bool dense_group3_rows(int64_t n);
int dense_small_group3(const float* const* in, const int64_t* n, const int32_t* const* n_dev, const float* const* W, float* const* out,
                       hipStream_t stream);
int dense_pack_frags(const float* W, int w_out_in, int cin, int cout, float* out, hipStream_t stream);

int bn_fold(const float* w, const float* b, const float* rm, const float* rv, float eps, int c, float* scale,
            float* shift, hipStream_t stream);
int gather_rows(const float* in, const int32_t* perm, int64_t n, int c, float* out, hipStream_t stream,
                const int32_t* n_dev = nullptr);
static constexpr int SEG_CHUNKS = 32;
int segment_partial_sums(const float* in, const int32_t* boff, int B, int c, int pow_mode, const float* p,
                         float* partial, hipStream_t stream);
int eca_apply(const float* x, const float* res, const float* partial, const int32_t* boff, int B, int64_t n, int c,
              const float* wconv, int ksize, float* out, hipStream_t stream);
int eca_gate_groups(const float* psum, const RowGroups& rg, const int32_t* boff, int B, int c, const float* wconv, int ksize,
                    float* gate, hipStream_t stream);
int eca_apply_gate(const void* x, const void* res, const float* gate, const int32_t* boff, int B, int64_t n, int c,
                   void* out, int bf16, hipStream_t stream);
int convert_bf16_to_f32(const void* in, int64_t n, float* out, hipStream_t stream);
int gem_finish(const float* partial, const int32_t* boff, int B, int c, const float* p, float* out,
               hipStream_t stream);
int pool_finish(const float* partial, const int32_t* boff, int B, int c, int mode, float* out, hipStream_t stream);
int l2_normalize_rows(float* x, int64_t n, int c, hipStream_t stream, const int32_t* n_dev = nullptr);
int add_act(const float* a, const float* b, int64_t n, int relu, float* out, hipStream_t stream);

constexpr int LH_WAVES = 8;
int keypoint_positions(const uint64_t* keys, int64_t n, int level, int cb, const float* offsets, int mode,
                       const float* step, int ignore_offsets, float* out, hipStream_t stream, const int32_t* n_dev = nullptr);
int local_heads_forward(const float* x, int64_t n, const int32_t* n_dev, const float* const* w, const uint64_t* keys,
                        int level, int cb, int mode, const float* step, int ignore_offsets, float* out_desc, float* out_kp,
                        float* out_sigma, hipStream_t stream, const float* lateral_w = nullptr, const float* lateral_res = nullptr,
                        int in_bf16 = 0, const void* split_pack = nullptr, int32_t* flags = nullptr);
size_t local_heads_pack_bytes();
int local_heads_pack(const float* const* w6_dev, void* out, hipStream_t stream);
int select_topk(const float* sigma, const int32_t* boff_dev, int B, int k, const float* kp, const float* desc, int dc,
                int32_t* sel_rows , int32_t* sel_count , float* out_kp, float* out_desc, hipStream_t stream);

static constexpr int NV_K = 64;
static constexpr int NV_MAX_CHUNKS = 32;
static constexpr int NV_CHUNK_ROWS = 128;
__host__ __device__ static inline int nv_chunks(int32_t len) {
  if (len <= 0) return 0;
  const int n = (len + NV_CHUNK_ROWS - 1) / NV_CHUNK_ROWS;
  return n < NV_MAX_CHUNKS ? n : NV_MAX_CHUNKS;
}
size_t netvlad_workspace_floats(int B, int C, int D);
void netvlad_workspace_carve(float* ws, int B, int C, float** part, float** vraw, float** sq, float** pp);
int netvlad_forward(const float* x, const int32_t* boff, int B, int C, const float* wc, const float* w2, const float* sc1,
                    const float* sh1, const float* H, int D, const float* sc2, const float* sh2, const float* wg,
                    const float* scg, const float* shg, int gating, float* out, float* ws, hipStream_t stream);

constexpr int LL_CLOUD_CHUNK = 1024;
constexpr int LL_STATS = 16;

}
```

egonn_amd/csrc/model.h:

```cpp
#pragma once
#include <map>
#include <string>
#include <vector>

#include "../../include/egonn_hip.h"
#include "common.h"
#include "kernels.h"

struct egonn_ctx : public egonn::Ctx {
  hipStream_t plan_stream = nullptr;

  void* level_feat[EGONN_NUM_LEVELS] = {};
  int level_ch[EGONN_NUM_LEVELS] = {};
  int level_bf16 = 0;
  bool from_points = false;
};

#define REQUIRE_PLAN(c)                                                                               \
  EGONN_REQUIRE((c) && (c)->plan.valid, EGONN_ERR_STATE, "no coordinate plan (call egonn_voxelize / " \
                                                         "egonn_coords_set first)")
#define REQUIRE_LEVEL(c, level)                                                                              \
  REQUIRE_PLAN(c);                                                                                           \
  HIP_CHECK(hipSetDevice((c)->device));                                                                      \
  EGONN_REQUIRE((level) >= 0 && (level) < EGONN_NUM_LEVELS, EGONN_ERR_INVALID, "level %d out of range", (level))

#define DBG_SYNC(...)                                                 \
  do {                                                                \
    if (switches().debug_sync) {                                      \
      fprintf(stderr, "[egonn] " __VA_ARGS__);                        \
      fprintf(stderr, "\n");                                          \
      fflush(stderr);                                                 \
      HIP_CHECK(hipStreamSynchronize(st));                            \
    }                                                                 \
  } while (0)

#define WALLOC(T, var, count)                                                      \
  T* var = A->alloc<T>((size_t)(count));                                           \
  EGONN_REQUIRE(var != nullptr, EGONN_ERR_STATE, "work arena too small (" #var ")")

namespace egonn {

int claim_work(egonn_ctx* c, size_t bytes, bool with_ksplit, Arena** A);

struct TensorRef {
  const float* p = nullptr;
  std::vector<int64_t> shape;
};

struct BnRef {
  const float *w = nullptr, *b = nullptr, *rm = nullptr, *rv = nullptr;
  float *scale = nullptr, *shift = nullptr;
  int c = 0;
};

struct BlockRef {
  const float *conv1 = nullptr, *conv2 = nullptr, *down = nullptr, *eca = nullptr;
  BnRef n1, n2, dn;
  int cin = 0, cout = 0, eca_k = 0;
};

struct MlpRef {
  const float *w0 = nullptr, *b0 = nullptr, *w1 = nullptr, *b1 = nullptr;
  int cin = 0, mid = 0, cout = 0;
};

struct ModelStore {
  enum Form { RG32, RG16, SPLIT, DENSE };
  struct Pack { Form form; const float* w; int K, ci, co; size_t off; const void** dst; };
  std::vector<BnRef*> bns;
  std::vector<Pack> packs;
  size_t bn_bytes = 0, pack_bytes = 0;
  char *folded = nullptr, *packed = nullptr;
  size_t folded_cap = 0, packed_cap = 0;

  void begin();
  void add_bn(BnRef* bn);
  void add_pack(Form form, const float* w, int K, int ci, int co, const void** dst);
  void add_kernel(const float* w, int K, int ci, int co, bool bf16, PackedKernel* dst);
  int commit(hipStream_t st);
  void release();
};

struct MinkFpnModel;
void minkfpn_model_free(MinkFpnModel* f);
void minkfpn_model_invalidate(MinkFpnModel* f);

}

struct egonn_model {
  std::map<std::string, egonn::TensorRef> t;
  bool ready = false;
  egonn::ModelStore store;
  const float* conv0 = nullptr;
  egonn::BnRef bn[8];
  const float* convs[8] = {};
  egonn::BlockRef blk[8];
  const float *g1x1[8] = {}, *gt[8] = {}, *l1x1[8] = {}, *lt[8] = {};
  const float* gem_p = nullptr;
  egonn::MlpRef gdec, ldec, kp, sg;
  void* conv0_unit = nullptr;
  void* lh_pack = nullptr;
  const float** lh_ptrs = nullptr;
  egonn::PackedKernel pk_convs[8], pk_c1[8], pk_c2[8], pk_gt[8], pk_lt[8];
  const void *pk_down[8] = {}, *pk_l1x1[8] = {};
  egonn::MinkFpnModel* fpn = nullptr;
};

namespace egonn {

int get_tensor(egonn_model* m, const std::string& key, std::initializer_list<int64_t> want, const float** out);
int get_bn(egonn_model* m, const std::string& prefix, int c, BnRef* bn, ModelStore* store);
int get_block(egonn_model* m, const std::string& prefix, int ci, int co, bool eca, BlockRef* b, ModelStore* store);
int eca_ksize(int c);
int conv_layer(egonn_ctx* c, hipStream_t st, const ConvCall& cc, const char* what);
ConvCall conv_call(int kind, int level, const void* in, const PackedKernel& pk, int cin, int cout, int bf16, const BnRef* bn, int relu,
                   void* out);
int ensure_graph_rowgroups(egonn_ctx* c, int L, const int* tlevels, int nt, hipStream_t st);
int block_convs(egonn_ctx* c, hipStream_t st, Arena* A, int level, const BlockRef& b, const PackedKernel& pk1, const PackedKernel& pk2,
                int bf16, const void* in, float* psum, void** t2);
DenseCall down_call(const BlockRef& b, const void* in, int bf16, int64_t n, const int32_t* n_dev, const void* wfrag);
int block_tail(const float* x, const float* res, const int32_t* boff, int B, int64_t n, int ch, const float* eca, int eca_k,
               float* partial, float* out, hipStream_t st);
enum Pooling { POOL_GEM = 1, POOL_MAC = 2, POOL_SPOC = 3 };
int global_pool(Pooling method, const float* x, const int32_t* boff, int B, int C, const float* p, float* partial, float* out,
                hipStream_t st);

bool topdown_split_supported(int C, int Cl);
int topdown_split_forward(Ctx* ctx, int level_out, const float* x_coarse, const void* sp_tconv, const float* x_lateral,
                          const void* sp_lateral, int C, int Cl, float* out, hipStream_t stream);

}
```

egonn_amd/csrc/model.hip:

```cpp
#include "model.h"

using namespace egonn;

namespace {

const int PLANES[7] = {32, 64, 64, 128, 128, 128, 128};
const int GLOBAL_CH = 128, GLOBAL_DIM = 256, LOCAL_CH = 64, LOCAL_DIM = 128;

}

API const char* egonn_last_error(void) { return last_error(); }

API int egonn_debug_set_naive_conv(egonn_ctx* c, int on) {
  EGONN_REQUIRE(c, EGONN_ERR_INVALID, "debug_set_naive_conv: null context");
  if (on >= 1000) { c->conv_variant = on; return EGONN_OK; }
  c->conv_variant = (on == 1) ? 3 : (on == 2 ? 1 : (on == 4 ? 2 : (on == 8 ? 4 : (on == 16 ? 5 : (on == 32 ? 6 : (on == 128 ? 9 : 0))))));
  return EGONN_OK;
}

API int egonn_debug_set_ksplit(egonn_ctx* c, int map_class, int level, int kparts, int kw, int col_parts) {
  EGONN_REQUIRE(c && (map_class == 0 || map_class == 1) && level >= 0 && level < EGONN_NUM_LEVELS, EGONN_ERR_INVALID,
                "debug_set_ksplit: bad argument");
  EGONN_REQUIRE(kparts <= 27 && kw <= 4 && col_parts <= 4, EGONN_ERR_INVALID, "debug_set_ksplit: kparts <= 27, kw <= 4, col_parts <= 4");
  if (kparts >= 0) c->ks_rule.kparts[map_class][level] = (int8_t)std::max(kparts, 1);
// ... 405 lines not shown
API int egonn_netvlad(egonn_ctx* c, int level, const float* x, int channels, const float* cluster_weights,
                      const float* cluster_weights2, const float* bn1_scale, const float* bn1_shift,
                      const float* hidden1_weights, const float* bn2_scale, const float* bn2_shift,
                      const float* gating_weights, const float* gate_scale, const float* gate_shift, int out_dim, int gating,
                      float* out, void* stream) {
  REQUIRE_PLAN(c);
  EGONN_REQUIRE(level >= 0 && level < EGONN_NUM_LEVELS, EGONN_ERR_INVALID, "netvlad: level %d out of range", level);
  EGONN_REQUIRE(channels >= 16 && channels <= 512 && channels % 16 == 0, EGONN_ERR_INVALID,
                "netvlad: %d channels unsupported (multiple of 16, 16..512)", channels);
  EGONN_REQUIRE(out_dim >= 16 && out_dim <= 1024 && out_dim % 16 == 0, EGONN_ERR_INVALID,
                "netvlad: output_dim %d unsupported (multiple of 16, 16..1024)", out_dim);
  EGONN_REQUIRE(x && cluster_weights && cluster_weights2 && bn1_scale && bn1_shift && hidden1_weights && bn2_scale &&
                    bn2_shift && out && (gating == 0 || gating == 1),
                EGONN_ERR_INVALID, "netvlad: bad argument");
  EGONN_REQUIRE(!gating || (gating_weights && gate_scale && gate_shift), EGONN_ERR_INVALID,
                "netvlad: gating needs gating_weights and the folded gate BatchNorm");
  EGONN_REQUIRE(((uintptr_t)x & 15) == 0, EGONN_ERR_INVALID, "netvlad: x must be 16-byte aligned");
  HIP_CHECK(hipSetDevice(c->device));
  const int B = c->plan.batch;
  const size_t nws = netvlad_workspace_floats(B, channels, out_dim);
  Arena* A;
  EGONN_TRY(claim_work(c, nws * 4 + 4096, false, &A));
  WALLOC(float, ws, nws);
  return netvlad_forward(x, c->plan.lv[level].boff, B, channels, cluster_weights, cluster_weights2, bn1_scale, bn1_shift,
                         hidden1_weights, out_dim, bn2_scale, bn2_shift, gating_weights, gate_scale, gate_shift, gating, out,
                         ws, (hipStream_t)stream);
}

API int egonn_model_create(egonn_model** m) {
  EGONN_REQUIRE(m, EGONN_ERR_INVALID, "model_create: null out pointer");
  *m = new egonn_model();
  return EGONN_OK;
}

API void egonn_model_destroy(egonn_model* m) {
  if (!m) return;
  m->store.release();
  if (m->conv0_unit) (void)hipFree(m->conv0_unit);
  if (m->lh_pack) (void)hipFree(m->lh_pack);
  if (m->lh_ptrs) (void)hipFree(m->lh_ptrs);
  if (m->fpn) minkfpn_model_free(m->fpn);
  delete m;
}

API int egonn_model_set_tensor(egonn_model* m, const char* key, const float* data, int ndim, const int64_t* shape) {
  EGONN_REQUIRE(m && key && data && ndim >= 0 && ndim <= 4, EGONN_ERR_INVALID, "model_set_tensor: bad argument");
  TensorRef r;
  r.p = data;
  r.shape.assign(shape, shape + ndim);
  m->t[key] = r;
  m->ready = false;
  if (m->fpn) minkfpn_model_invalidate(m->fpn);
  return EGONN_OK;
}

namespace egonn {

int get_tensor(egonn_model* m, const std::string& key, std::initializer_list<int64_t> want, const float** out) {
  auto it = m->t.find(key);
  EGONN_REQUIRE(it != m->t.end(), EGONN_ERR_STATE, "model: missing state_dict tensor '%s'", key.c_str());
  const std::vector<int64_t>& s = it->second.shape;
  bool ok = s.size() == want.size();
  size_t i = 0;
  for (int64_t w : want) {
    if (ok && s[i] != w) ok = false;
    ++i;
  }
  if (!ok) {
    std::string got = "(", exp = "(";
    for (int64_t v : s) got += std::to_string(v) + ",";
    for (int64_t v : want) exp += std::to_string(v) + ",";
    set_error("model: tensor '%s' has shape %s), expected %s)", key.c_str(), got.c_str(), exp.c_str());
    return EGONN_ERR_INVALID;
  }
  *out = it->second.p;
  return EGONN_OK;
}

int get_bn(egonn_model* m, const std::string& prefix, int c, BnRef* bn, ModelStore* store) {
  bn->c = c;
  EGONN_TRY(get_tensor(m, prefix + ".bn.weight", {c}, &bn->w));
  EGONN_TRY(get_tensor(m, prefix + ".bn.bias", {c}, &bn->b));
  EGONN_TRY(get_tensor(m, prefix + ".bn.running_mean", {c}, &bn->rm));
  EGONN_TRY(get_tensor(m, prefix + ".bn.running_var", {c}, &bn->rv));
  store->add_bn(bn);
  return EGONN_OK;
}

int eca_ksize(int c) {
  int lg = 0;
  while ((1 << lg) < c) ++lg;
  const int t = (lg + 1) / 2;
  return (t % 2) ? t : t + 1;
}

int get_block(egonn_model* m, const std::string& prefix, int ci, int co, bool eca, BlockRef* b, ModelStore* store) {
  *b = BlockRef();
  b->cin = ci;
  b->cout = co;
  EGONN_TRY(get_tensor(m, prefix + ".conv1.kernel", {27, ci, co}, &b->conv1));
  EGONN_TRY(get_bn(m, prefix + ".norm1", co, &b->n1, store));
  EGONN_TRY(get_tensor(m, prefix + ".conv2.kernel", {27, co, co}, &b->conv2));
  EGONN_TRY(get_bn(m, prefix + ".norm2", co, &b->n2, store));
  if (ci != co) {
    EGONN_TRY(get_tensor(m, prefix + ".downsample.0.kernel", {ci, co}, &b->down));
    EGONN_TRY(get_bn(m, prefix + ".downsample.1", co, &b->dn, store));
  }
  if (eca) {
    b->eca_k = eca_ksize(co);
    EGONN_TRY(get_tensor(m, prefix + ".eca.conv.weight", {1, 1, b->eca_k}, &b->eca));
  }
  return EGONN_OK;
}

void ModelStore::begin() {
  bns.clear();
  packs.clear();
  bn_bytes = pack_bytes = 0;
}
void ModelStore::add_bn(BnRef* bn) {
  bns.push_back(bn);
  bn_bytes += align_up((size_t)2 * bn->c * sizeof(float), 256);
}
void ModelStore::add_pack(Form form, const float* w, int K, int ci, int co, const void** dst) {
  packs.push_back({form, w, K, ci, co, pack_bytes, dst});
  const size_t n = (size_t)K * ci * co;
  pack_bytes += align_up(form == SPLIT ? split_weights_bytes(K, ci, co) : form == RG16 ? n * 2 : n * 4, 256);
}
void ModelStore::add_kernel(const float* w, int K, int ci, int co, bool bf16, PackedKernel* dst) {
  *dst = PackedKernel();
  add_pack(RG32, w, K, ci, co, &dst->rg32);
  if (bf16) add_pack(RG16, w, K, ci, co, &dst->rg16);
  if (sconv_split_supported(ci, co)) add_pack(SPLIT, w, K, ci, co, &dst->split);
}
int ModelStore::commit(hipStream_t st) {
  auto grow = [](char** buf, size_t* cap, size_t need) -> int {
    if (*cap >= need) return EGONN_OK;
    if (*buf) HIP_CHECK(hipFree(*buf));
    *buf = nullptr;
    *cap = 0;
    HIP_CHECK(hipMalloc(reinterpret_cast<void**>(buf), need));
    *cap = need;
    return EGONN_OK;
  };
  EGONN_TRY(grow(&folded, &folded_cap, bn_bytes));
  EGONN_TRY(grow(&packed, &packed_cap, pack_bytes));
  for (const Pack& k : packs) {
    char* out = packed + k.off;
    switch (k.form) {
      case RG32: EGONN_TRY(pack_rg_weights(k.w, k.K, k.ci, k.co, 0, 0, 0, out, st)); break;
      case RG16: EGONN_TRY(pack_rg_weights(k.w, k.K, k.ci, k.co, 1, 0, 0, out, st)); break;
      case SPLIT: EGONN_TRY(pack_split_weights(k.w, k.K, k.ci, k.co, 0, 0, out, st)); break;
      case DENSE: EGONN_TRY(dense_pack_frags(k.w, 0, k.ci, k.co, reinterpret_cast<float*>(out), st)); break;
    }
    *k.dst = out;
  }
  char* cur = folded;
  for (BnRef* bn : bns) {
    bn->scale = reinterpret_cast<float*>(cur);
    bn->shift = bn->scale + bn->c;
    cur += align_up((size_t)2 * bn->c * sizeof(float), 256);
    EGONN_TRY(bn_fold(bn->w, bn->b, bn->rm, bn->rv, 1e-5f, bn->c, bn->scale, bn->shift, st));
  }
  return EGONN_OK;
}
void ModelStore::release() {
  if (folded) (void)hipFree(folded);
  if (packed) (void)hipFree(packed);
  folded = packed = nullptr;
  folded_cap = packed_cap = 0;
}

}

namespace {

int get_mlp(egonn_model* m, const std::string& prefix, int cin, int mid, int cout, MlpRef* r) {
  r->cin = cin; r->mid = mid; r->cout = cout;
  EGONN_TRY(get_tensor(m, prefix + ".net.0.linear.weight", {mid, cin}, &r->w0));
  EGONN_TRY(get_tensor(m, prefix + ".net.0.linear.bias", {mid}, &r->b0));
  EGONN_TRY(get_tensor(m, prefix + ".net.2.linear.weight", {cout, mid}, &r->w1));
  EGONN_TRY(get_tensor(m, prefix + ".net.2.linear.bias", {cout}, &r->b1));
  return EGONN_OK;
}

}

API int egonn_model_finalize(egonn_model* m, void* stream) {
  EGONN_REQUIRE(m, EGONN_ERR_INVALID, "model_finalize: null model");
  hipStream_t st = (hipStream_t)stream;
  ModelStore& S = m->store;
  S.begin();
  auto dense = [&](const float* w, int ci, int co, const void** dst) {
    *dst = nullptr;
    if (ci % 16 == 0 && co % 16 == 0) S.add_pack(ModelStore::DENSE, w, 1, ci, co, dst);
  };
  EGONN_TRY(get_tensor(m, "trunk.convs.0.kernel", {125, 1, 32}, &m->conv0));
  EGONN_TRY(get_bn(m, "trunk.bn.0", 32, &m->bn[0], &S));
  int inpl = PLANES[0];
  for (int i = 1; i <= 7; ++i) {
    const std::string si = std::to_string(i);
    const int cout = PLANES[i - 1];
    EGONN_TRY(get_tensor(m, "trunk.convs." + si + ".kernel", {8, inpl, inpl}, &m->convs[i]));
    EGONN_TRY(get_bn(m, "trunk.bn." + si, inpl, &m->bn[i], &S));
    BlockRef& b = m->blk[i];
    EGONN_TRY(get_block(m, "trunk.blocks." + si + ".0", inpl, cout, true, &b, &S));
    S.add_kernel(m->convs[i], 8, inpl, inpl, true, &m->pk_convs[i]);
    S.add_kernel(b.conv1, 27, inpl, cout, true, &m->pk_c1[i]);
    S.add_kernel(b.conv2, 27, cout, cout, true, &m->pk_c2[i]);
    m->pk_down[i] = nullptr;
    if (b.down) dense(b.down, inpl, cout, &m->pk_down[i]);
    inpl = cout;
  }
  for (int l : {5, 6, 7})
    EGONN_TRY(get_tensor(m, "global_head.conv1x1." + std::to_string(l) + ".kernel", {PLANES[l - 1], GLOBAL_CH}, &m->g1x1[l]));
  for (int l : {6, 7}) {
    EGONN_TRY(get_tensor(m, "global_head.tconv." + std::to_string(l) + ".kernel", {8, GLOBAL_CH, GLOBAL_CH}, &m->gt[l]));
    S.add_kernel(m->gt[l], 8, GLOBAL_CH, GLOBAL_CH, true, &m->pk_gt[l]);
  }
  for (int l : {3, 4}) {
    EGONN_TRY(get_tensor(m, "local_head.conv1x1." + std::to_string(l) + ".kernel", {PLANES[l - 1], LOCAL_CH}, &m->l1x1[l]));
    dense(m->l1x1[l], PLANES[l - 1], LOCAL_CH, &m->pk_l1x1[l]);
  }
  EGONN_TRY(get_tensor(m, "local_head.tconv.4.kernel", {8, LOCAL_CH, LOCAL_CH}, &m->lt[4]));
  S.add_kernel(m->lt[4], 8, LOCAL_CH, LOCAL_CH, true, &m->pk_lt[4]);
  m->gem_p = nullptr;
  if (m->t.count("global_pooling.pooling.p")) EGONN_TRY(get_tensor(m, "global_pooling.pooling.p", {1}, &m->gem_p));
  EGONN_TRY(get_mlp(m, "global_descriptor_decoder", GLOBAL_CH, GLOBAL_DIM + (GLOBAL_CH - GLOBAL_DIM) / 2, GLOBAL_DIM, &m->gdec));
  EGONN_TRY(get_mlp(m, "local_descriptor_decoder", LOCAL_CH, LOCAL_DIM + (LOCAL_CH - LOCAL_DIM) / 2, LOCAL_DIM, &m->ldec));
  EGONN_TRY(get_mlp(m, "local_keypoint_regressor", LOCAL_CH, LOCAL_CH / 2, 3, &m->kp));
  EGONN_TRY(get_mlp(m, "local_sigma_regressor", LOCAL_CH, LOCAL_CH / 2, 1, &m->sg));

  EGONN_TRY(S.commit(st));
  if (!m->conv0_unit) HIP_CHECK(hipMalloc(&m->conv0_unit, 2 * 4 * 3 * 64 * 16));
  EGONN_TRY(conv0_pack_unit(m->conv0, m->conv0_unit, st));
  if (m->ldec.cin == 64 && m->ldec.mid == 96 && m->ldec.cout == 128 && m->kp.mid == 32 && m->sg.mid == 32 && m->kp.cin == 64 &&
      m->sg.cin == 64) {
    if (!m->lh_pack) HIP_CHECK(hipMalloc(&m->lh_pack, local_heads_pack_bytes()));
    if (!m->lh_ptrs) HIP_CHECK(hipMalloc(reinterpret_cast<void**>(&m->lh_ptrs), 6 * sizeof(float*)));
    const float* hp[6] = {m->ldec.w0, m->ldec.w1, m->kp.w0, m->kp.w1, m->sg.w0, m->sg.w1};
    HIP_CHECK(hipMemcpyAsync(m->lh_ptrs, hp, sizeof(hp), hipMemcpyHostToDevice, st));
    HIP_CHECK(hipStreamSynchronize(st));
    EGONN_TRY(local_heads_pack(m->lh_ptrs, m->lh_pack, st));
  }
  m->ready = true;
  return EGONN_OK;
}

namespace {

int run_mlp(const MlpRef& r, const float* x, int64_t n, int act_out, float* hidden, float* out, hipStream_t st,
            const int32_t* n_dev) {
  EGONN_TRY(dense_forward({.in = x, .n = n, .n_dev = n_dev, .cin = r.cin, .cout = r.mid, .W = r.w0, .w_out_in = 1, .bias = r.b0,
                           .act = ACT_RELU, .out = hidden},
                          st));
  return dense_forward({.in = hidden, .n = n, .n_dev = n_dev, .cin = r.mid, .cout = r.cout, .W = r.w1, .w_out_in = 1, .bias = r.b1,
                        .act = act_out, .out = out},
                       st);
}

}

namespace egonn {

int claim_work(egonn_ctx* c, size_t bytes, bool with_ksplit, Arena** A) {
  for (int l = 0; l < EGONN_NUM_LEVELS; ++l) c->level_feat[l] = nullptr;
  c->ks_part = nullptr;
  c->ks_part_floats = 0;
  EGONN_TRY(c->work_arena.ensure(bytes));
  c->work_arena.reset();
  *A = &c->work_arena;
  const size_t ks = with_ksplit ? sconv_ksplit_scratch_floats(c) : 0;
  if (ks) {
    c->ks_part = (*A)->alloc<float>(ks);
    EGONN_REQUIRE(c->ks_part, EGONN_ERR_STATE, "work arena too small (ks_part)");
    c->ks_part_floats = ks;
  }
  return EGONN_OK;
}

int conv_layer(egonn_ctx* c, hipStream_t st, const ConvCall& cc, const char* what) {
  static const int pk[3] = {PK_K3, PK_K2S2, PK_TCONV};
  char tag[64];
  snprintf(tag, sizeof(tag), "%s<%d,%d>/L%d/%s", sconv_kernel_name(c, cc.kind, cc.level, cc.cin, cc.cout, cc.bf16), cc.cin, cc.cout,
           cc.level, what);
  ProfScope ps(c, st, tag, pk[cc.kind], cc.level, cc.kind == 0 ? 27 : 8, cc.cin, cc.cout, cc.bf16 ? 2 : 4);
  return sconv_map(c, cc, st);
}
ConvCall conv_call(int kind, int level, const void* in, const PackedKernel& pk, int cin, int cout, int bf16, const BnRef* bn, int relu,
                   void* out) {
  return ConvCall{.kind = kind, .level = level, .in = in, .out = out, .cin = cin, .cout = cout, .bf16 = bf16,
                  .scale = bn ? bn->scale : nullptr, .shift = bn ? bn->shift : nullptr, .relu = relu, .packed = &pk};
}

int ensure_graph_rowgroups(egonn_ctx* c, int L, const int* tlevels, int nt, hipStream_t st) {
  int kinds[RG_MAX_JOBS], levels[RG_MAX_JOBS], n = 0;
  for (int l = 1; l <= L; ++l) { kinds[n] = 0; levels[n++] = l; }
  for (int l = 1; l <= L; ++l) { kinds[n] = 1; levels[n++] = l; }
  for (int i = 0; i < nt; ++i) { kinds[n] = 2; levels[n++] = tlevels[i]; }
  return ensure_rowgroups(c, kinds, levels, n, st);
}

int block_convs(egonn_ctx* c, hipStream_t st, Arena* A, int level, const BlockRef& b, const PackedKernel& pk1, const PackedKernel& pk2,
                int bf16, const void* in, float* psum, void** t2_out) {
  const size_t bytes = (size_t)c->plan.cap[level] * b.cout * (bf16 ? 2 : 4);
  WALLOC(char, t1, bytes);
  WALLOC(char, t2, bytes);
  const bool t1_split = !switches().no_presplit && sconv_route(c, 0, level, b.cin, b.cout, bf16) == ROUTE_SPLIT &&
                        sconv_route(c, 0, level, b.cout, b.cout, bf16) == ROUTE_SPLIT;
  ConvCall c1 = conv_call(0, level, in, pk1, b.cin, b.cout, bf16, &b.n1, 1, t1);
  c1.split_io = t1_split ? 2 : 0;
  EGONN_TRY(conv_layer(c, st, c1, "k3.conv1"));
  ConvCall c2 = conv_call(0, level, t1, pk2, b.cout, b.cout, bf16, &b.n2, 0, t2);
  c2.split_io = t1_split ? 1 : 0;
  c2.psum = psum;
  EGONN_TRY(conv_layer(c, st, c2, "k3.conv2"));
  *t2_out = t2;
  return EGONN_OK;
}

DenseCall down_call(const BlockRef& b, const void* in, int bf16, int64_t n, const int32_t* n_dev, const void* wfrag) {
  return DenseCall{.in = in, .in_bf16 = bf16, .n = n, .n_dev = n_dev, .cin = b.cin, .cout = b.cout, .W = b.down,
                   .wfrag = static_cast<const float*>(wfrag), .scale = b.dn.scale, .shift = b.dn.shift, .out_bf16 = bf16};
}

int global_pool(Pooling method, const float* x, const int32_t* boff, int B, int C, const float* p, float* partial, float* out,
                hipStream_t st) {
  if (method == POOL_GEM) {
    EGONN_TRY(segment_partial_sums(x, boff, B, C, 1, p, partial, st));
    return gem_finish(partial, boff, B, C, p, out, st);
  }
  const int mode = method == POOL_MAC ? 2 : 0;
  EGONN_TRY(segment_partial_sums(x, boff, B, C, mode, nullptr, partial, st));
  return pool_finish(partial, boff, B, C, mode, out, st);
}

int block_tail(const float* x, const float* res, const int32_t* boff, int B, int64_t n, int ch, const float* eca, int eca_k,
               float* partial, float* out, hipStream_t st) {
  if (!eca) return add_act(x, res, n * ch, 1, out, st);
  EGONN_TRY(segment_partial_sums(x, boff, B, ch, 0, nullptr, partial, st));
  return eca_apply(x, res, partial, boff, B, n, ch, eca, eca_k, out, st);
}

}

API int egonn_forward(egonn_ctx* c, egonn_model* m, const float* features, int quant_mode, const float* step, int flags,
                      float* out_global, float* out_desc, float* out_kp, float* out_sigma, void* stream) {
  REQUIRE_PLAN(c);
  EGONN_REQUIRE(m && m->ready, EGONN_ERR_STATE, "model not finalized (call egonn_model_finalize)");
  EGONN_REQUIRE(step, EGONN_ERR_INVALID, "forward: null argument");
  HIP_CHECK(hipSetDevice(c->device));
  hipStream_t st = (hipStream_t)stream;
  Plan& P = c->plan;
  const int B = P.batch;
  const int32_t* cnt = c->dev_counts;
  const int bf16 = (flags & EGONN_FLAG_BF16) ? 1 : 0;
  const size_t es = bf16 ? 2 : 4;
  const bool do_global = !(flags & EGONN_FLAG_DISABLE_GLOBAL);
  const bool do_local = !(flags & EGONN_FLAG_DISABLE_LOCAL);
  EGONN_REQUIRE(!do_global || out_global, EGONN_ERR_INVALID, "forward: out_global is null");
  EGONN_REQUIRE(!do_local || (out_desc && out_kp && out_sigma), EGONN_ERR_INVALID, "forward: local outputs are null");
  HIP_CHECK(hipMemsetAsync(c->dev_fp16_flag, 0, sizeof(int32_t), st));

  {
    const int tlevels[3] = {6, 5, 3};
    EGONN_TRY(ensure_graph_rowgroups(c, 7, tlevels + (do_global ? 0 : 2), (do_global ? 2 : 0) + (do_local ? 1 : 0), st));
    DBG_SYNC("row groups");
  }

  size_t need = (size_t)P.cap[0] * (1 + 32) * 4;
  for (int i = 1; i <= 7; ++i) need += (size_t)P.cap[i] * 128 * 4 * 6 + (size_t)P.lv[i].rg27.cap_groups * 128 * 4;
  need += (size_t)P.cap[5] * (192 + 256 + 128 * 2) * 4 + (size_t)P.cap[3] * (96 + 32 + 32 + 3 + 64 * 2) * 4;
  need += (size_t)B * SEG_CHUNKS * 256 * 4 * 10 + (size_t)P.cap[3] * 32 + (4u << 20);
  need += sconv_ksplit_scratch_floats(c) * 4 + 4096;
  Arena* A;
  EGONN_TRY(claim_work(c, need, true, &A));

  const int64_t n0 = P.cap[0];
  const float* f0 = features;
  if (features && !c->from_points) {
    WALLOC(float, fg, n0);
    EGONN_TRY(gather_rows(features, P.perm0, n0, 1, fg, st, cnt));
    f0 = fg;
  }
  WALLOC(char, x0, n0 * 32 * es);
  {
    ProfScope ps(c, st, "conv0_k5_kernel/L0", PK_CONV0, 0, 125, 1, 32, (int)es);
    EGONN_TRY(conv0_k5_forward(c, f0, m->conv0, 32, m->bn[0].scale, m->bn[0].shift, 1, x0, bf16, st, m->conv0_unit));
  }
  DBG_SYNC("conv0");
  const void* x[8] = {x0};
  c->level_feat[0] = x0;
  c->level_ch[0] = 32;
  c->level_bf16 = bf16;
  auto local_head = [&](hipStream_t st) -> int {
    const int64_t n3 = P.cap[3], n4 = P.cap[4];
    WALLOC(char, l4, n4 * LOCAL_CH * es);
    EGONN_TRY(dense_forward({.in = x[4], .in_bf16 = bf16, .n = n4, .n_dev = cnt + 4, .cin = 128, .cout = LOCAL_CH, .W = m->l1x1[4],
                             .wfrag = static_cast<const float*>(m->pk_l1x1[4]), .out = l4, .out_bf16 = bf16},
                            st));
    WALLOC(char, u3, n3 * LOCAL_CH * es);
    EGONN_TRY(conv_layer(c, st, conv_call(2, 3, l4, m->pk_lt[4], LOCAL_CH, LOCAL_CH, bf16, nullptr, 0, u3), "tconv"));
    EGONN_REQUIRE(m->ldec.cin == 64 && m->ldec.mid == 96 && m->ldec.cout == 128 && m->kp.mid == 32 && m->sg.mid == 32,
                  EGONN_ERR_STATE, "local heads: unexpected layer sizes");
    const float* hw[12] = {m->ldec.w0, m->ldec.b0, m->ldec.w1, m->ldec.b1, m->kp.w0, m->kp.b0, m->kp.w1, m->kp.b1,
                           m->sg.w0, m->sg.b0, m->sg.w1, m->sg.b1};
    const void* lh_pack = (!switches().no_split_heads && sconv_split_arithmetic(c)) ? m->lh_pack : nullptr;
    if (!switches().no_fused_lateral && LOCAL_CH == 64) {
      EGONN_TRY(local_heads_forward(reinterpret_cast<const float*>(x[3]), n3, cnt + 3, hw, P.lv[3].keys, 3, P.coord_bits, quant_mode,
                                    step, (flags & EGONN_FLAG_IGNORE_KP_REGRESSOR) ? 1 : 0, out_desc, out_kp, out_sigma, st,
                                    m->l1x1[3], reinterpret_cast<const float*>(u3), bf16, lh_pack, c->dev_fp16_flag));
      return EGONN_OK;
    }
    WALLOC(float, l3, n3 * LOCAL_CH);
    EGONN_TRY(dense_forward({.in = x[3], .in_bf16 = bf16, .n = n3, .n_dev = cnt + 3, .cin = 64, .cout = LOCAL_CH, .W = m->l1x1[3],
                             .wfrag = static_cast<const float*>(m->pk_l1x1[3]), .residual = u3, .res_bf16 = bf16, .out = l3},
                            st));
    EGONN_TRY(local_heads_forward(l3, n3, cnt + 3, hw, P.lv[3].keys, 3, P.coord_bits, quant_mode, step,
                                  (flags & EGONN_FLAG_IGNORE_KP_REGRESSOR) ? 1 : 0, out_desc, out_kp, out_sigma, st, nullptr, nullptr, 0,
                                  lh_pack, c->dev_fp16_flag));
    return EGONN_OK;
  };
  const float *gated_t2 = nullptr, *gated_res = nullptr, *gated_gate = nullptr;
  for (int i = 1; i <= 7; ++i) {
    const BlockRef& b = m->blk[i];
    const Level& L = P.lv[i];
    const int64_t n = P.cap[i];
    WALLOC(char, y, n * b.cin * es);
    {
      ConvCall cc = conv_call(1, i, x[i - 1], m->pk_convs[i], b.cin, b.cin, bf16, &m->bn[i], 1, y);
      if (gated_t2 && i == 2) {
        cc.in = gated_t2;
        cc.in2 = gated_res;
        cc.gate = gated_gate;
      }
      EGONN_TRY(conv_layer(c, st, cc, "k2s2"));
    }
    DBG_SYNC("L%d k2s2", i);
    WALLOC(float, psum, (size_t)L.rg27.cap_groups * b.cout);
    void* t2 = nullptr;
    EGONN_TRY(block_convs(c, st, A, i, b, m->pk_c1[i], m->pk_c2[i], bf16, y, psum, &t2));
    WALLOC(float, gate, (size_t)B * b.cout);
    DBG_SYNC("L%d convs", i);
    EGONN_TRY(eca_gate_groups(psum, L.rg27, L.boff, B, b.cout, b.eca, b.eca_k, gate, st));
    DBG_SYNC("L%d eca gate", i);
    const void* res = y;
    if (i == 1 && !switches().no_gated_k2s2 && !c->keep_level_features && !bf16 && !b.down && c->conv_variant == 0 && b.cout == 32 &&
        m->blk[2].cin == 32 && sconv_route(c, 1, 2, 32, 32, 0) == ROUTE_SPLIT) {
      gated_t2 = reinterpret_cast<const float*>(t2);
      gated_res = reinterpret_cast<const float*>(y);
      gated_gate = gate;
      x[i] = nullptr;
      c->level_feat[i] = nullptr;
      c->level_ch[i] = b.cout;
      continue;
    }
    WALLOC(char, xo, n * b.cout * es);
    const DenseCall down = down_call(b, y, bf16, n, cnt + i, m->pk_down[i]);
    if (b.down && !switches().no_fused_down && dense_gate_fusable(n, b.cin, b.cout)) {
      DenseCall dc = down;
      dc.residual = t2; dc.res_bf16 = bf16;
      dc.gate = gate; dc.boff = L.boff; dc.B = B;
      dc.out = xo;
      EGONN_TRY(dense_forward(dc, st));
    } else {
      if (b.down) {
        WALLOC(char, rd, n * b.cout * es);
        DenseCall dc = down;
        dc.out = rd;
        EGONN_TRY(dense_forward(dc, st));
        res = rd;
      }
      EGONN_TRY(eca_apply_gate(t2, res, gate, L.boff, B, n, b.cout, xo, bf16, st));
    }
    DBG_SYNC("L%d eca apply", i);
    x[i] = xo;
    c->level_feat[i] = xo;
    c->level_ch[i] = b.cout;
  }
  if (do_local) EGONN_TRY(local_head(st));
  DBG_SYNC("local head");

  void* g5_fused = nullptr;
  if (do_global && !switches().no_fused_ghead && !bf16 && c->conv_variant == 0 && dense_group3_rows(P.cap[5]) &&
      dense_group3_rows(P.cap[6]) && dense_group3_rows(P.cap[7])) {
    WALLOC(float, l7, P.cap[7] * GLOBAL_CH);
    WALLOC(float, l6, P.cap[6] * GLOBAL_CH);
    WALLOC(float, l5, P.cap[5] * GLOBAL_CH);
    WALLOC(float, g6f, P.cap[6] * GLOBAL_CH);
    WALLOC(float, g5f, P.cap[5] * GLOBAL_CH);
    const float* gin[3] = {reinterpret_cast<const float*>(x[7]), reinterpret_cast<const float*>(x[6]), reinterpret_cast<const float*>(x[5])};
    const int64_t gn[3] = {P.cap[7], P.cap[6], P.cap[5]};
    const int32_t* gnd[3] = {cnt + 7, cnt + 6, cnt + 5};
    const float* gw[3] = {m->g1x1[7], m->g1x1[6], m->g1x1[5]};
    float* gout[3] = {l7, l6, l5};
    EGONN_TRY(dense_small_group3(gin, gn, gnd, gw, gout, st));
    for (int lv = 6; lv >= 5; --lv) {
      ConvCall cc = conv_call(2, lv, lv == 6 ? l7 : g6f, m->pk_gt[lv + 1], GLOBAL_CH, GLOBAL_CH, 0, nullptr, 0, lv == 6 ? g6f : g5f);
      cc.residual = lv == 6 ? l6 : l5;
      EGONN_TRY(conv_layer(c, st, cc, "tconv"));
    }
    g5_fused = g5f;
    DBG_SYNC("global head (fused)");
  }
  if (do_global) {
    const float* g5 = reinterpret_cast<const float*>(g5_fused);
    if (!g5) {
    auto lateral = [&](int l, const void* up, void* out, int out_bf16) {
      return dense_forward({.in = x[l], .in_bf16 = bf16, .n = P.cap[l], .n_dev = cnt + l, .cin = 128, .cout = GLOBAL_CH, .W = m->g1x1[l],
                            .residual = up, .res_bf16 = up ? bf16 : 0, .out = out, .out_bf16 = out_bf16},
                           st);
    };
    WALLOC(char, g7, P.cap[7] * GLOBAL_CH * es);
    EGONN_TRY(lateral(7, nullptr, g7, bf16));
    WALLOC(char, u6, P.cap[6] * GLOBAL_CH * es);
    EGONN_TRY(conv_layer(c, st, conv_call(2, 6, g7, m->pk_gt[7], GLOBAL_CH, GLOBAL_CH, bf16, nullptr, 0, u6), "tconv"));
    WALLOC(char, g6, P.cap[6] * GLOBAL_CH * es);
    EGONN_TRY(lateral(6, u6, g6, bf16));
    WALLOC(char, u5, P.cap[5] * GLOBAL_CH * es);
    EGONN_TRY(conv_layer(c, st, conv_call(2, 5, g6, m->pk_gt[6], GLOBAL_CH, GLOBAL_CH, bf16, nullptr, 0, u5), "tconv"));
    WALLOC(float, g5u, P.cap[5] * GLOBAL_CH);
    EGONN_TRY(lateral(5, u5, g5u, 0));
    g5 = g5u;
    DBG_SYNC("global head");
    }
    WALLOC(float, gh, P.cap[5] * m->gdec.mid);
    WALLOC(float, gd, P.cap[5] * GLOBAL_DIM);
    EGONN_TRY(run_mlp(m->gdec, g5, P.cap[5], ACT_NONE, gh, gd, st, cnt + 5));
    WALLOC(float, gp, (size_t)B * SEG_CHUNKS * GLOBAL_DIM);
    const Pooling pool = (flags & EGONN_FLAG_POOL_MAC) ? POOL_MAC : (flags & EGONN_FLAG_POOL_SPOC) ? POOL_SPOC : POOL_GEM;
    EGONN_REQUIRE(pool != POOL_GEM || m->gem_p, EGONN_ERR_STATE, "forward: GeM pooling needs the tensor 'global_pooling.pooling.p'");
    EGONN_TRY(global_pool(pool, gd, P.lv[5].boff, B, GLOBAL_DIM, m->gem_p, gp, out_global, st));
  }

  DBG_SYNC("global decoder + pooling");
  return EGONN_OK;
}

API int egonn_forward_level_features(egonn_ctx* c, int level, float* out, int channels, void* stream) {
  REQUIRE_PLAN(c);
  EGONN_REQUIRE(level >= 0 && level < EGONN_NUM_LEVELS && c->level_feat[level], EGONN_ERR_STATE,
                "no features for level %d (run egonn_forward first; level 1 of fp32 maps is materialised only after "
                "egonn_debug_keep_level_features(ctx, 1))", level);
  EGONN_REQUIRE(channels == c->level_ch[level], EGONN_ERR_INVALID, "level %d has %d channels, caller expects %d", level,
                c->level_ch[level], channels);
  const int64_t cnt = c->plan.lv[level].n * channels;
  if (c->level_bf16) return convert_bf16_to_f32(c->level_feat[level], cnt, out, (hipStream_t)stream);
  HIP_CHECK(hipMemcpyAsync(out, c->level_feat[level], sizeof(float) * cnt, hipMemcpyDeviceToDevice, (hipStream_t)stream));
  return EGONN_OK;
}

API int egonn_select_keypoints(egonn_ctx* c, const float* sigma, const float* keypoints, const float* descriptors,
                               int n_k, float* sel_kp, float* sel_desc, int32_t* sel_rows, int32_t* sel_count,
                               void* stream) {
  REQUIRE_PLAN(c);
  EGONN_REQUIRE(sigma && keypoints && descriptors && sel_kp && sel_desc && sel_rows && sel_count, EGONN_ERR_INVALID,
                "select_keypoints: null argument");
  HIP_CHECK(hipSetDevice(c->device));
  return select_topk(sigma, c->plan.lv[3].boff, c->plan.batch, n_k, keypoints, descriptors, LOCAL_DIM, sel_rows, sel_count,
                     sel_kp, sel_desc, (hipStream_t)stream);
}


API int egonn_topk_rows(const float* sigma, const int32_t* row_offsets, int batch_size, int n_k, int32_t* sel_rows,
                        int32_t* sel_count, void* stream) {
  EGONN_REQUIRE(sigma && row_offsets && sel_rows && sel_count && batch_size >= 1, EGONN_ERR_INVALID, "topk_rows: bad argument");
  return select_topk(sigma, row_offsets, batch_size, n_k, nullptr, nullptr, 0, sel_rows, sel_count, nullptr, nullptr,
                     (hipStream_t)stream);
}

API int egonn_profile_enable(egonn_ctx* c, int mode, const char* filter) {
  EGONN_REQUIRE(c && mode >= 0 && mode <= 3, EGONN_ERR_INVALID, "profile_enable: bad argument");
  c->prof.mode = mode;
  snprintf(c->prof.filter, sizeof(c->prof.filter), "%s", filter ? filter : "");
  return EGONN_OK;
}

API int egonn_profile_fetch(egonn_ctx* c, int cap, int* n, char* names, float* ms, double* bytes, double* flops,
                            void* stream) {
  EGONN_REQUIRE(c && n && names && ms && bytes && flops, EGONN_ERR_INVALID, "profile_fetch: null argument");
  HIP_CHECK(hipSetDevice(c->device));
  Plan& P = c->plan;
  if (P.valid) {
    if (P.built_reserved) P.exact = false;
    EGONN_TRY(plan_sync(c, (hipStream_t)stream));
    EGONN_TRY(count_map_pairs(c, (hipStream_t)stream));
  }
  HIP_CHECK(hipStreamSynchronize((hipStream_t)stream));
  unsigned long long pairs[16];
  HIP_CHECK(hipMemcpy(pairs, c->dev_pairs, sizeof(pairs), hipMemcpyDeviceToHost));
  int w = 0;
  std::vector<ProfRec> all(c->prof.recs);
  all.insert(all.end(), c->prof.graph_recs.begin(), c->prof.graph_recs.end());
  const size_t n_plain = c->prof.recs.size();
  size_t ri = 0;
  for (auto& r : all) {
    const bool plain = ri++ < n_plain;
    float t = 0.f;
    if (hipEventSynchronize(r.e1) != hipSuccess || hipEventElapsedTime(&t, r.e0, r.e1) != hipSuccess) {
      (void)hipGetLastError();
      if (plain) { c->prof.pool.push_back(r.e0); c->prof.pool.push_back(r.e1); }
      continue;
    }
    if (w < cap) {
      const double n_out = (double)P.lv[r.level].n;
      double Pn = 0;
      switch (r.kind) {
        case PK_CONV0: Pn = (double)pairs[0]; break;
        case PK_K3: Pn = (double)pairs[r.level]; break;
        case PK_K2S2: Pn = (double)P.lv[r.level - 1].n; break;
        case PK_TCONV: Pn = n_out; break;
        default: Pn = n_out; break;
      }
      snprintf(names + (size_t)w * 64, 64, "%s", r.name);
      ms[w] = t;
      bytes[w] = Pn * r.cin * r.es + n_out * r.cout * r.es + (double)r.K * r.cin * r.cout * r.es + 8.0 * Pn;
      flops[w] = 2.0 * Pn * r.cin * r.cout;
      ++w;
    }
    if (plain) { c->prof.pool.push_back(r.e0); c->prof.pool.push_back(r.e1); }
  }
  c->prof.recs.clear();
  *n = w;
  return EGONN_OK;
}
```

include/egonn_hip.h:

```cpp
#ifndef EGONN_HIP_H
#define EGONN_HIP_H

#include <stdint.h>

#ifdef __cplusplus
extern "C" {
#endif

typedef struct egonn_ctx egonn_ctx;
typedef struct egonn_model egonn_model;

enum { EGONN_QUANT_CARTESIAN = 0, EGONN_QUANT_POLAR = 1 };
enum { EGONN_STATUS_OK = 0, EGONN_STATUS_INVALID = 1, EGONN_STATUS_HIP = 2, EGONN_STATUS_RANGE = 3, EGONN_STATUS_STATE = 4,
       EGONN_STATUS_CAPACITY = 5,
       EGONN_STATUS_FP16_RANGE = 6 };
enum { EGONN_FLAG_DISABLE_GLOBAL = 1, EGONN_FLAG_DISABLE_LOCAL = 2, EGONN_FLAG_IGNORE_KP_REGRESSOR = 4,
       EGONN_FLAG_BF16 = 8,
       EGONN_FLAG_POOL_SPOC = 16, EGONN_FLAG_POOL_MAC = 32 };

int egonn_ctx_create(egonn_ctx** ctx, int device, int coord_bits);
void egonn_ctx_destroy(egonn_ctx* ctx);
const char* egonn_last_error(void);
int egonn_debug_set_naive_conv(egonn_ctx* ctx, int on);
int egonn_debug_set_ksplit(egonn_ctx* ctx, int map_class, int level, int kparts, int kw, int col_parts);
int egonn_debug_set_resident(egonn_ctx* ctx, int mask, int max_workgroups);
int egonn_debug_keep_level_features(egonn_ctx* ctx, int on);
int egonn_debug_set_trace(void* device_buffer);
int egonn_debug_rowgroup_tables(egonn_ctx* ctx, int map_kind, int level_out, uint32_t* gmask_out, int32_t* snbr_out,
                                int64_t capacity_groups, int64_t* n_groups, void* stream);
int egonn_debug_rowgroup_perm(egonn_ctx* ctx, int map_kind, int level_out, int32_t* perm_out, int64_t capacity_groups,
                              int64_t* n_groups, void* stream);
int64_t egonn_debug_radix_sort_scratch_bytes(int64_t n, int n_segments);
int egonn_debug_radix_sort(uint64_t* keys_in, uint32_t* vals_in, uint64_t* keys_out, uint32_t* vals_out, int64_t n, int nbits,
                           const int64_t* n_dev, const int64_t* seg_offsets, int n_segments, int idx_bits, int either_pair,
                           int32_t* result_pair, void* scratch, int64_t scratch_bytes, void* stream);

int egonn_voxelize(egonn_ctx* ctx, const float* points, const int64_t* scan_offsets, int batch_size, int quant_mode,
                   const float* step, void* stream);
int egonn_ctx_reserve(egonn_ctx* ctx, int64_t max_points, int batch_size, const int64_t* level_capacity);
int egonn_voxelize_device(egonn_ctx* ctx, const float* points, int64_t n_rows, const int64_t* scan_offsets_dev,
                          int batch_size, int quant_mode, const float* step, void* stream);
int egonn_plan_status(egonn_ctx* ctx, void* stream);
int egonn_ctx_set_exact_fp32(egonn_ctx* ctx, int on);
int egonn_ctx_set_operand_autoscale(egonn_ctx* ctx, int on);
int egonn_level_capacity(egonn_ctx* ctx, int level, int64_t* capacity);
typedef struct egonn_graph egonn_graph;
int egonn_graph_begin(void* stream);
int egonn_graph_end(void* stream, egonn_graph** graph);
int egonn_graph_launch(egonn_graph* graph, void* stream);
void egonn_graph_destroy(egonn_graph* graph);
int egonn_coords_set(egonn_ctx* ctx, const int32_t* coords, int64_t n, int batch_size, void* stream);

int egonn_level_count(egonn_ctx* ctx, int level, int64_t* n_rows);
int egonn_level_batch_offsets(egonn_ctx* ctx, int level, int64_t* offsets );
int egonn_level_coords(egonn_ctx* ctx, int level, int32_t* out, void* stream);
int egonn_input_index(egonn_ctx* ctx, int64_t* out , void* stream);

int egonn_conv(egonn_ctx* ctx, int level_in, int level_out, int kernel_size, const float* in, int cin,
               const float* kernel, int cout, const float* scale, const float* shift, int relu, float* out,
               void* stream);
int egonn_conv_transpose(egonn_ctx* ctx, int level_in, const float* in, int cin, const float* kernel, int cout,
                         float* out, void* stream);
int egonn_sparse_conv(egonn_ctx* ctx, int map_kind, int level_out, const void* in, int cin, const float* kernel, int cout,
                      int bf16, const float* scale, const float* shift, int relu, void* out, float* group_sums,
                      void* stream);
int egonn_prepare_maps(egonn_ctx* ctx, int with_level0_transpose, void* stream);
int egonn_map_groups(egonn_ctx* ctx, int map_kind, int level_out, int64_t* n_groups, int64_t* first_group, void* stream);
int egonn_global_avg_pool(egonn_ctx* ctx, int level, const float* in, int channels, float* out, void* stream);

int egonn_bn_fold(const float* weight, const float* bias, const float* running_mean, const float* running_var,
                  float eps, int channels, float* scale, float* shift, void* stream);
int egonn_block_tail(egonn_ctx* ctx, int level, const float* x, const float* residual, int channels,
                     const float* eca_weight, int eca_ksize, float* out, void* stream);
int egonn_add(const float* a, const float* b, int64_t n, float* out, void* stream);
int egonn_gather_input(egonn_ctx* ctx, const float* features, int channels, float* out, void* stream);
int egonn_gem(egonn_ctx* ctx, int level, const float* x, int channels, const float* p, float* out, void* stream);
int egonn_global_max_pool(egonn_ctx* ctx, int level, const float* in, int channels, float* out, void* stream);
int egonn_netvlad(egonn_ctx* ctx, int level, const float* x, int channels, const float* cluster_weights,
                  const float* cluster_weights2, const float* bn1_scale, const float* bn1_shift,
                  const float* hidden1_weights, const float* bn2_scale, const float* bn2_shift,
                  const float* gating_weights, const float* gate_scale, const float* gate_shift, int out_dim, int gating,
                  float* out, void* stream);
int egonn_netvlad_train_forward(egonn_ctx* ctx, int level, const float* x, int channels, int nmax,
                                const float* cluster_weights, const float* cluster_weights2, const float* bn1_weight,
                                const float* bn1_bias, float bn1_eps, float bn1_momentum, float* bn1_running_mean,
                                float* bn1_running_var, const float* hidden1_weights, int out_dim, float* out, float* save_z,
                                float* save_bn1, float* save_v, float* save_sq, float* save_asum, void* stream);
int egonn_netvlad_train_backward(egonn_ctx* ctx, int level, const float* x, int channels, int nmax,
                                 const float* cluster_weights, const float* cluster_weights2, const float* bn1_weight,
                                 const float* hidden1_weights, int out_dim, const float* grad_out, const float* save_z,
                                 const float* save_bn1, const float* save_v, const float* save_sq, const float* save_asum,
                                 float* grad_x, float* grad_cluster_weights, float* grad_cluster_weights2, float* out_bn1,
                                 float* grad_hidden1_weights, void* stream);
int egonn_global_max_pool_argmax(egonn_ctx* ctx, int level, const float* in, int channels, float* out, int32_t* out_rows,
                                 void* stream);
int egonn_global_max_pool_backward(egonn_ctx* ctx, int level, const float* grad_out, const int32_t* rows, int channels,
                                   float* grad_in, void* stream);
int egonn_sigmoid_gate(const float* y, const float* t, const float* grad_out, int64_t n, float* out, float* grad_y,
                       float* grad_t, void* stream);

int egonn_model_create(egonn_model** model);
void egonn_model_destroy(egonn_model* model);
int egonn_model_set_tensor(egonn_model* model, const char* key, const float* data, int ndim, const int64_t* shape);
int egonn_model_finalize(egonn_model* model, void* stream);

int egonn_forward(egonn_ctx* ctx, egonn_model* model, const float* features, int quant_mode, const float* step,
                  int flags, float* out_global, float* out_descriptors, float* out_keypoints, float* out_sigma,
                  void* stream);
int egonn_forward_level_features(egonn_ctx* ctx, int level, float* out, int channels, void* stream);

int egonn_minkfpn_finalize(egonn_model* model, int n_levels, const int* planes, const int* layers, int num_top_down,
                           int feature_size, int block, int pooling, void* stream);
int egonn_minkfpn_out_level(int n_levels, int num_top_down, int* level);
enum { EGONN_MINKFPN_SPLIT_TOPDOWN = 1 };
int egonn_minkfpn_forward(egonn_ctx* ctx, egonn_model* model, int flags, float* out_global, float* out_map, void* stream);
int egonn_topdown_step(egonn_ctx* ctx, int level_out, const float* x_coarse, const float* w_tconv, const float* x_lateral,
                       const float* w_lateral, int C, int Cl, float* out, void* stream);

int egonn_select_keypoints(egonn_ctx* ctx, const float* sigma, const float* keypoints, const float* descriptors,
                           int n_k, float* sel_keypoints, float* sel_descriptors, int32_t* sel_rows,
                           int32_t* sel_count, void* stream);

int egonn_topk_rows(const float* sigma, const int32_t* row_offsets, int batch_size, int n_k, int32_t* sel_rows,
                    int32_t* sel_count, void* stream);

int64_t egonn_triplet_loss_scratch_floats(int n);
int egonn_triplet_loss(const float* embeddings, int n, int d, const uint8_t* positives_mask,
                       const uint8_t* negatives_mask, float margin, float* out_stats, int32_t* out_triplets,
                       float* out_grad, float* scratch, void* stream);

int64_t egonn_contrastive_loss_scratch_floats(int n);
int egonn_contrastive_loss(const float* embeddings, int n, int d, const uint8_t* positives_mask,
                           const uint8_t* negatives_mask, float pos_margin, float neg_margin, float* out_stats,
                           int32_t* out_triplets, float* out_grad, float* scratch, void* stream);

int egonn_nn_search(const float* a, int64_t n, const float* transform, const float* b, int64_t m, float* out_dist,
                    int32_t* out_index, void* stream);
int egonn_matrix_min(const float* d, int64_t n, int64_t m, float* row_min, int32_t* row_index, float* col_min,
                     int32_t* col_index, void* stream);
int egonn_softmax_cross_entropy(const float* logits, int64_t n, int64_t m, const int32_t* target, float* out_loss,
                                int32_t* out_argmax, float* out_dlogits, void* stream);

#define EGONN_LOCAL_LOSS_STATS 16
enum { EGONN_LL_LOSS = 0, EGONN_LL_KP_PER_CLOUD = 1, EGONN_LL_REPEATABILITY = 2, EGONN_LL_CHAMFER_PURE = 3,
       EGONN_LL_CHAMFER_WEIGHTED = 4, EGONN_LL_MEAN_SIGMA = 5, EGONN_LL_LOSS_CHAMFER = 6, EGONN_LL_LOSS_P2P = 7,
       EGONN_LL_KEYPOINT_LOSS = 8, EGONN_LL_CORRESPONDENCE_LOSS = 9, EGONN_LL_MATCHING_KEYPOINTS = 10,
       EGONN_LL_MATCHING_DESCRIPTORS = 11, EGONN_LL_POS_SIMILARITY = 12, EGONN_LL_NEG_SIMILARITY = 13  };
int64_t egonn_local_loss_scratch_bytes(int pairs, int64_t n_kp1, int64_t n_kp2, int dim);
int egonn_local_loss(int pairs, int64_t n_cloud1, int64_t n_cloud2, int64_t n_kp1, int64_t n_kp2, int dim,
                     const float* clouds1, const int32_t* cloud_off1, const float* clouds2, const int32_t* cloud_off2,
                     const float* kp1, const float* sigma1, const float* desc1, const int32_t* kp_off1,
                     const float* kp2, const float* sigma2, const float* desc2, const int32_t* kp_off2,
                     const float* transforms, const float* params, float* out_pair, float* out_batch,
                     float* g_kp1, float* g_sigma1, float* g_desc1, float* g_kp2, float* g_sigma2, float* g_desc2,
                     void* scratch, int64_t scratch_bytes, void* stream);

enum { EGONN_ACT_NONE = 0, EGONN_ACT_RELU = 1, EGONN_ACT_TANH = 2, EGONN_ACT_SOFTPLUS = 3, EGONN_ACT_SIGMOID = 4 };
int egonn_dense(const float* x, int64_t n, int cin, const float* weight, int weight_out_in, const float* bias, int cout,
                int act, float* out, void* stream);
int egonn_dense_pack_fragments(const float* weight, int weight_out_in, int cin, int cout, float* packed, void* stream);
int egonn_dense_pack_fragments_host(const float* weight, int weight_out_in, int cin, int cout, float* packed);
int egonn_debug_dense(const void* in, int in_bf16, int64_t rows_capacity, const int32_t* n_dev, int cin, int cout, const float* weight,
                      int weight_out_in, const float* packed, const float* bias, const float* scale, const float* shift, int act,
                      const void* residual, int res_bf16, const float* gate, const int32_t* boff, int B, void* out, int out_bf16,
                      int form, void* stream);
int egonn_debug_dense_route(int64_t rows, int cin, int cout, int form, int gate_scans, int32_t out[5]);
int egonn_dense_backward_weight(const float* a, int ca, const float* b, int cb, int64_t n, float* out, float* scratch,
                                int64_t scratch_floats, void* stream);
int egonn_conv_backward_weight(egonn_ctx* ctx, int level_in, int level_out, int kernel_size, int transposed,
                               const float* in, int cin, const float* grad_out, int cout, float* grad_kernel,
                               float* scratch, int64_t scratch_floats, void* stream);
int egonn_col_stats(int mode, const float* a, const float* b, const float* mask, const float* mean, int64_t n, int c,
                    double* out, float* scratch, int64_t scratch_floats, void* stream);
int egonn_bn_train_finalize(const double* sums, const float* shift_point, double count, int c, const float* weight,
                            const float* bias, float eps, float momentum, float* running_mean, float* running_var,
                            float* out_mean_invstd_scale_shift, void* stream);
int egonn_bn_backward_finalize(const double* local_sums, const double* global_sums, double count, int c, const float* weight,
                               const float* mean, const float* invstd, float* out_abc_dgamma_dbeta, void* stream);
int egonn_affine_act(const float* x, const float* scale, const float* shift, int64_t n, int c, int relu, float* out,
                     void* stream);
int egonn_affine3(const float* g, const float* mask, const float* x, const float* A, const float* B, const float* C,
                  int64_t n, int c, float* out, void* stream);
int egonn_relu_backward(const float* grad_out, const float* out, int64_t n, int c, float* grad_in, void* stream);
int egonn_act_backward(int act, const float* grad_out, const float* out, int64_t n, int c, float* grad_in, void* stream);
int egonn_l2_normalize(const float* x, const float* grad_out, int64_t n, int c, float* out, void* stream);
int egonn_eca_gate(const float* mean, const float* conv_weight, int kernel_size, int batch_size, int channels, float* gate,
                   void* stream);
int egonn_eca_gate_backward(const float* grad_gate, const float* gate, const float* mean, const float* conv_weight,
// ... 150 lines not shown
```

Before: 22760.

## Fuse global decoder MLP with pooling partials and pack lateral weights

Adds a fused kernel that runs the two-layer global decoder MLP (128->192->256) with MFMA on row tiles held in shared memory, and accumulates pooling partial sums directly. This avoids writing the hidden and output activations to global memory and drops separate launches. It also switches the grouped lateral 1x1 dense launch to use pre-packed weight fragments, and staggers B-fragment loads in the small dense body to lower register pressure for wide inputs. The fused tail launches only SEG_CHUNKS x B blocks, so it may use few workgroups and lose parallelism at small batch.

```diff
diff --git a/egonn_amd/_lib.py b/egonn_amd/_lib.py
--- a/egonn_amd/_lib.py
+++ b/egonn_amd/_lib.py
@@ -33,6 +33,9 @@
     ("egonn_debug_radix_sort_scratch_bytes", C.c_int64, [C.c_int64, C.c_int]),
     ("egonn_debug_radix_sort", C.c_int, [_P, _P, _P, _P, C.c_int64, C.c_int, _P, _P, C.c_int, C.c_int, C.c_int,
                                          C.POINTER(C.c_int32), _P, C.c_int64, _P]),
+    ("egonn_debug_dense_group3", C.c_int, [_P, _P, _P, _P, _P, _P, _P]),
+    ("egonn_debug_global_tail_scratch_bytes", C.c_int64, [C.c_int64]),
+    ("egonn_debug_global_tail", C.c_int, [_P, _P, C.c_int, C.c_int64, _P, _P, _P, _P, _P, _P, C.c_int, C.c_int, _P, _P, _P, C.c_int64, _P]),
     ("egonn_voxelize", C.c_int, [_P, _P, C.POINTER(C.c_int64), C.c_int, C.c_int, C.POINTER(C.c_float), _P]),
     ("egonn_ctx_reserve", C.c_int, [_P, C.c_int64, C.c_int, C.POINTER(C.c_int64)]),
     ("egonn_voxelize_device", C.c_int, [_P, _P, C.c_int64, _P, C.c_int, C.c_int, C.POINTER(C.c_float), _P]),
@@ -315,6 +318,36 @@
     return pair.value
 
 
+def debug_dense_group3(xs, capacities, counts, ws, packed: bool):
+    lib = load()
+    dev = xs[0].device
+    arr = lambda ptrs: (C.c_void_p * 3)(*ptrs)
+    nds = [torch.tensor([int(c)], dtype=torch.int32, device=dev) for c in counts]
+    pks = [dense_pack_fragments(w, False) for w in ws] if packed else [None] * 3
+    bufs = [torch.full((max(int(c), 1), 128), -12345.0, dtype=torch.float32, device=dev) for c in capacities]
+    call(dev, lib.egonn_debug_dense_group3, arr([x.data_ptr() for x in xs]), (C.c_int64 * 3)(*[int(c) for c in capacities]),
+         arr([n.data_ptr() for n in nds]), arr([w.data_ptr() for w in ws]), arr([_ptr(p) for p in pks]),
+         arr([b.data_ptr() for b in bufs]))
+    return [b[:int(c)] for b, c in zip(bufs, capacities)]
+
+
+GLOBAL_TAIL_POOLING = {"GeM": 1, "MAC": 2, "SPoC": 3}
+
+
+def debug_global_tail(g5, row_offsets, n_dev, w0, b0, w1, b1, p, pooling: str, form: int):
+    lib = load()
+    B = row_offsets.numel() - 1
+    cap = g5.shape[0]
+    need = lib.egonn_debug_global_tail_scratch_bytes(int(cap))
+    buf = scratch(need, g5.device)
+    partial = torch.empty((B, 32, 256), dtype=torch.float32, device=g5.device)
+    out = torch.empty((B, 256), dtype=torch.float32, device=g5.device)
+    call(g5.device, lib.egonn_debug_global_tail, g5.data_ptr(), row_offsets.data_ptr(), B, int(cap), n_dev.data_ptr(), w0.data_ptr(),
+         b0.data_ptr(), w1.data_ptr(), b1.data_ptr(), _ptr(p), GLOBAL_TAIL_POOLING[pooling], int(form), partial.data_ptr(),
+         out.data_ptr(), buf.data_ptr(), need)
+    return partial, out
+
+
 def require_gpu() -> torch.device:
     if not torch.cuda.is_available():
         raise RuntimeError("egonn_amd: no HIP device visible (torch.cuda.is_available() is False); "
diff --git a/egonn_amd/csrc/common.h b/egonn_amd/csrc/common.h
--- a/egonn_amd/csrc/common.h
+++ b/egonn_amd/csrc/common.h
@@ -202,6 +202,8 @@
   bool no_fused_lateral;
   bool no_gated_k2s2;
   bool no_fused_ghead;
+  bool no_fused_gtail;
+  bool no_packed_laterals;
   bool no_split_heads;
   bool no_tail_split;
   bool no_task_order;
diff --git a/egonn_amd/csrc/coords.hip b/egonn_amd/csrc/coords.hip
--- a/egonn_amd/csrc/coords.hip
+++ b/egonn_amd/csrc/coords.hip
@@ -21,7 +21,8 @@
     const char* ds = getenv("EGONN_DEBUG_SYNC");
     return Switches{.debug_sync = ds && ds[0] == '1', .no_presplit = on("EGONN_NO_PRESPLIT"), .no_fused_down = on("EGONN_NO_FUSED_DOWN"),
                     .no_fused_lateral = on("EGONN_NO_FUSED_LATERAL"), .no_gated_k2s2 = on("EGONN_NO_GATED_K2S2"),
-                    .no_fused_ghead = on("EGONN_NO_FUSED_GHEAD"), .no_split_heads = on("EGONN_NO_SPLIT_HEADS"),
+                    .no_fused_ghead = on("EGONN_NO_FUSED_GHEAD"), .no_fused_gtail = on("EGONN_NO_FUSED_GTAIL"),
+                    .no_packed_laterals = on("EGONN_NO_PACKED_LATERALS"), .no_split_heads = on("EGONN_NO_SPLIT_HEADS"),
                     .no_tail_split = on("EGONN_NO_TAIL_SPLIT"), .no_task_order = on("EGONN_NO_TASK_ORDER"),
                     .flat_sort = on("EGONN_FLAT_SORT"), .sort_pairs = on("EGONN_SORT_PAIRS"), .no_search67 = on("EGONN_NO_SEARCH67"),
                     .no_dense_stream = on("EGONN_NO_DENSE_STREAM"),
diff --git a/egonn_amd/csrc/dense.hip b/egonn_amd/csrc/dense.hip
--- a/egonn_amd/csrc/dense.hip
+++ b/egonn_amd/csrc/dense.hip
@@ -100,7 +100,7 @@
 }
 
 template <int W_OUT_IN, int CIN, bool IN_BF16>
-__device__ static inline void dense_small_body(const void* __restrict__ in_v, int64_t n,
+__device__ static inline __attribute__((always_inline)) void dense_small_body(const void* __restrict__ in_v, int64_t n,
                                                const float* __restrict__ W, int cout,
                                                const float* __restrict__ bias, const float* __restrict__ scale,
                                                const float* __restrict__ shift, int act,
@@ -134,26 +134,33 @@
   const float* bias_p = bias ? bias : W;
   const float* scale_p = scale ? scale : W;
   const float* shift_p = scale ? shift : W;
+  auto load_b = [&](int nt) {
+    const int col = min(ncol0 + nt * 16 + l15, cout - 1);
+#pragma unroll
+    for (int t = 0; t < KS; ++t) {
+      float4 v;
+      if (W_OUT_IN == 2) {
+        v = *reinterpret_cast<const float4*>(W + ((int64_t)((col >> 4) * KS + t) * 64 + lane) * 4);
+      } else if (W_OUT_IN == 1) {
+        v = *reinterpret_cast<const float4*>(W + (int64_t)col * CIN + 16 * t + 4 * g4);
+      } else {
+        const uint32_t uc = (uint32_t)cout, o = (uint32_t)(16 * t + 4 * g4) * uc + (uint32_t)col;
+        v.x = W[o];
+        v.y = W[o + uc];
+        v.z = W[o + 2u * uc];
+        v.w = W[o + 3u * uc];
+      }
+      b[nt][t] = v;
+    }
+  };
+  constexpr int NUP = (CIN >= 128 && !IN_BF16 && W_OUT_IN == 0) ? 3 : 4;
 #pragma unroll
   for (int nt = 0; nt < 4; ++nt) {
     const int col = min(ncol0 + nt * 16 + l15, cout - 1);
     bi[nt] = bias_p[col];
     sc[nt] = scale_p[col];
     sh[nt] = shift_p[col];
-#pragma unroll
-    for (int t = 0; t < KS; ++t) {
-      float4 v;
-      if (W_OUT_IN) {
-        v = *reinterpret_cast<const float4*>(W + (int64_t)col * CIN + 16 * t + 4 * g4);
-      } else {
-        const float* wp = W + (int64_t)(16 * t + 4 * g4) * cout + col;
-        v.x = wp[0];
-        v.y = wp[cout];
-        v.z = wp[2 * (int64_t)cout];
-        v.w = wp[3 * (int64_t)cout];
-      }
-      b[nt][t] = v;
-    }
+    if (nt < NUP) load_b(nt);
   }
   float res[4][4];
   {
@@ -188,6 +195,10 @@
   for (int nt = 0; nt < 4; ++nt) {
     const int col = ncol0 + nt * 16 + l15;
     if (ncol0 + nt * 16 >= cout) break;
+    if constexpr (NUP < 4) {
+      if (nt >= 1 && nt + NUP - 1 < 4) load_b(nt + NUP - 1);
+      __builtin_amdgcn_sched_barrier(0);
+    }
     f32x4 acc = {0.f, 0.f, 0.f, 0.f};
 #pragma unroll
     for (int t = 0; t < KS; ++t) {
@@ -631,18 +642,20 @@
 }
 
 bool dense_group3_rows(int64_t n) { return n == 0 || dense_route(n, 128, 128, -1) == DENSE_SMALL; }
-int dense_small_group3(const float* const* in, const int64_t* n, const int32_t* const* n_dev, const float* const* W, float* const* out,
-                       hipStream_t stream) {
+int dense_small_group3(const float* const* in, const int64_t* n, const int32_t* const* n_dev, const float* const* W,
+                       const float* const* wfrag, float* const* out, hipStream_t stream) {
+  const bool packed = wfrag && wfrag[0] && wfrag[1] && wfrag[2];
   DenseGroup3 g;
   int bx = 0;
   for (int q = 0; q < 3; ++q) {
     EGONN_REQUIRE(dense_group3_rows(n[q]), EGONN_ERR_INVALID, "dense(group): %lld rows", (long long)n[q]);
-    g.in[q] = in[q]; g.W[q] = W[q]; g.out[q] = out[q]; g.n_dev[q] = n_dev[q]; g.n[q] = n[q];
+    g.in[q] = in[q]; g.W[q] = packed ? wfrag[q] : W[q]; g.out[q] = out[q]; g.n_dev[q] = n_dev[q]; g.n[q] = n[q];
     g.bx0[q] = bx;
     bx += (int)cdiv(std::max<int64_t>(n[q], 1), 64);
   }
   g.bx0[3] = bx;
-  hipLaunchKernelGGL((dense_small3_kernel<0, 128, false>), dim3((unsigned)bx, 2), dim3(256), 0, stream, g, 128, 0);
+  if (packed) hipLaunchKernelGGL((dense_small3_kernel<2, 128, false>), dim3((unsigned)bx, 2), dim3(256), 0, stream, g, 128, 0);
+  else hipLaunchKernelGGL((dense_small3_kernel<0, 128, false>), dim3((unsigned)bx, 2), dim3(256), 0, stream, g, 128, 0);
   HIP_CHECK(hipGetLastError());
   return EGONN_OK;
 }
@@ -681,6 +694,17 @@
                         .out_bf16 = out_bf16 ? 1 : 0, .form = form},
                        (hipStream_t)stream);
 }
+API int egonn_debug_dense_group3(const float* const in[3], const int64_t rows_capacity[3], const int32_t* const n_dev[3],
+                                 const float* const weight[3], const float* const packed[3], float* const out[3], void* stream) {
+  EGONN_REQUIRE(in && rows_capacity && n_dev && weight && packed && out, EGONN_ERR_INVALID, "debug_dense_group3: null argument");
+  for (int q = 0; q < 3; ++q) {
+    EGONN_REQUIRE(in[q] && n_dev[q] && weight[q] && out[q] && rows_capacity[q] >= 0 && !packed[q] == !packed[0], EGONN_ERR_INVALID,
+                  "debug_dense_group3: bad arguments of problem %d", q);
+    EGONN_REQUIRE(dense_group3_rows(rows_capacity[q]), EGONN_ERR_INVALID, "debug_dense_group3: %lld rows are not a small launch",
+                  (long long)rows_capacity[q]);
+  }
+  return dense_small_group3(in, rows_capacity, n_dev, weight, packed, out, (hipStream_t)stream);
+}
 API int egonn_debug_dense_route(int64_t rows, int cin, int cout, int form, int gate_scans, int32_t out[5]) {
   EGONN_REQUIRE(out && rows >= 0 && cin >= 1 && cout >= 1 && form >= -1 && form <= 1 && gate_scans >= 0, EGONN_ERR_INVALID,
                 "debug_dense_route: bad arguments");
diff --git a/egonn_amd/csrc/global_tail.hip b/egonn_amd/csrc/global_tail.hip
--- /dev/null
+++ b/egonn_amd/csrc/global_tail.hip
@@ -0,0 +1,106 @@
+#include "common.h"
+#include "kernels.h"
+#include "rowmath.h"
+
+namespace egonn {
+
+constexpr int GT_KS0 = GTAIL_CIN / 16, GT_KS1 = GTAIL_MID / 16;
+constexpr int GT_NT0 = GTAIL_MID / 16 / 4, GT_NT1 = GTAIL_OUT / 16 / 4;
+constexpr int GT_HS = GTAIL_MID + 4, GT_OS = GTAIL_OUT + 4;
+
+__global__ __launch_bounds__(256, 2) void global_tail_kernel(const float* __restrict__ g5, int64_t ncap, const int32_t* __restrict__ boff,
+                                                             const f32x4* __restrict__ wf0, const float* __restrict__ b0,
+                                                             const f32x4* __restrict__ wf1, const float* __restrict__ b1, int pow_mode,
+                                                             const float* __restrict__ pexp, float* __restrict__ partial) {
+  __shared__ __attribute__((aligned(16))) float s_hid[16 * GT_HS];
+  __shared__ __attribute__((aligned(16))) float s_out[16 * GT_OS];
+  const int b = blockIdx.y, ch = blockIdx.x;
+  const int32_t s = boff[b], e = boff[b + 1];
+  const int64_t len = e - s;
+  const int32_t r0 = s + (int32_t)(len * ch / SEG_CHUNKS);
+  const int32_t r1 = ncap > 0 ? s + (int32_t)(len * (ch + 1) / SEG_CHUNKS) : r0;
+  const int tid = threadIdx.x, lane = tid & 63, wave = tid >> 6;
+  const int l15 = lane & 15, g4 = lane >> 4;
+  const float p = pow_mode == 1 ? pexp[0] : 1.f;
+  float run = pow_mode == 2 ? -INFINITY : 0.f;
+#pragma unroll 1
+  for (int32_t base = r0; base < r1; base += 16) {
+    int zero = 0;
+    asm volatile("" : "+s"(zero));
+    const f32x4* const w0p = wf0 + (int64_t)wave * GT_NT0 * GT_KS0 * 64 + lane + zero;
+    const f32x4* const w1p = wf1 + (int64_t)wave * GT_NT1 * GT_KS1 * 64 + lane + zero;
+    const int64_t row = max(min((int64_t)min(base + l15, r1 - 1), ncap - 1), (int64_t)0);
+    f32x4 a[GT_KS0], w0[GT_NT0][GT_KS0], w1[2][GT_KS1];
+    float bh[GT_NT0];
+#pragma unroll
+    for (int t = 0; t < GT_KS0; ++t) a[t] = *reinterpret_cast<const f32x4*>(g5 + row * GTAIL_CIN + 16 * t + 4 * g4);
+#pragma unroll
+    for (int j = 0; j < GT_NT0; ++j) {
+#pragma unroll
+      for (int t = 0; t < GT_KS0; ++t) w0[j][t] = w0p[(j * GT_KS0 + t) * 64];
+      bh[j] = b0[16 * (wave * GT_NT0 + j) + l15];
+    }
+#pragma unroll
+    for (int t = 0; t < GT_KS1; ++t) w1[0][t] = w1p[t * 64];
+    __builtin_amdgcn_sched_barrier(0);
+#pragma unroll
+    for (int j = 0; j < GT_NT0; ++j) {
+      f32x4 acc = {0.f, 0.f, 0.f, 0.f};
+#pragma unroll
+      for (int t = 0; t < GT_KS0; ++t) {
+#pragma unroll
+        for (int u = 0; u < 4; ++u) acc = __builtin_amdgcn_mfma_f32_16x16x4f32(a[t][u], w0[j][t][u], acc, 0, 0, 0);
+      }
+#pragma unroll
+      for (int r = 0; r < 4; ++r) s_hid[(4 * g4 + r) * GT_HS + 16 * (wave * GT_NT0 + j) + l15] = fmaxf(acc[r] + bh[j], 0.f);
+      __builtin_amdgcn_sched_barrier(0);
+    }
+    __syncthreads();
+    f32x4 h[GT_KS1];
+#pragma unroll
+    for (int t = 0; t < GT_KS1; ++t) h[t] = *reinterpret_cast<const f32x4*>(s_hid + l15 * GT_HS + 16 * t + 4 * g4);
+    __builtin_amdgcn_sched_barrier(0);
+#pragma unroll
+    for (int j = 0; j < GT_NT1; ++j) {
+      const int c0 = 16 * (wave * GT_NT1 + j) + 4 * g4;
+      const f32x4 bo = *reinterpret_cast<const f32x4*>(b1 + c0);
+      if (j + 1 < GT_NT1) {
+#pragma unroll
+        for (int t = 0; t < GT_KS1; ++t) w1[(j + 1) & 1][t] = w1p[((j + 1) * GT_KS1 + t) * 64];
+      }
+      f32x4 acc = {0.f, 0.f, 0.f, 0.f};
+#pragma unroll
+      for (int t = 0; t < GT_KS1; ++t) {
+#pragma unroll
+        for (int u = 0; u < 4; ++u) acc = __builtin_amdgcn_mfma_f32_16x16x4f32(w1[j & 1][t][u], h[t][u], acc, 0, 0, 0);
+      }
+      f32x4 v = acc + bo;
+      v = v * 1.f + 0.f;
+      *reinterpret_cast<f32x4*>(s_out + l15 * GT_OS + c0) = v;
+      __builtin_amdgcn_sched_barrier(0);
+    }
+    __syncthreads();
+    const int nrows = min(16, r1 - base);
+    for (int r = 0; r < nrows; ++r) {
+      float v = s_out[r * GT_OS + tid];
+      if (pow_mode == 1) v = powf(fmaxf(v, 1e-6f), p);
+      run = pow_mode == 2 ? fmaxf(run, v) : run + v;
+    }
+  }
+  float sum = pow_mode == 2 ? -INFINITY : 0.f;
+  sum = pow_mode == 2 ? fmaxf(sum, run) : sum + run;
+  partial[((int64_t)b * SEG_CHUNKS + ch) * GTAIL_OUT + tid] = sum;
+}
+
+int global_tail_fused(const float* g5, int64_t ncap, const int32_t* boff, int B, const float* wf0, const float* b0, const float* wf1,
+                      const float* b1, int pow_mode, const float* p, float* partial, hipStream_t stream) {
+  EGONN_REQUIRE(g5 && boff && wf0 && b0 && wf1 && b1 && partial && B >= 1 && ncap >= 0 && pow_mode >= 0 && pow_mode <= 2 &&
+                    (pow_mode != 1 || p),
+                EGONN_ERR_INVALID, "global tail: bad arguments");
+  hipLaunchKernelGGL(global_tail_kernel, dim3(SEG_CHUNKS, B), dim3(256), 0, stream, g5, ncap, boff, reinterpret_cast<const f32x4*>(wf0),
+                     b0, reinterpret_cast<const f32x4*>(wf1), b1, pow_mode, p, partial);
+  HIP_CHECK(hipGetLastError());
+  return EGONN_OK;
+}
+
+}
diff --git a/egonn_amd/csrc/kernels.h b/egonn_amd/csrc/kernels.h
--- a/egonn_amd/csrc/kernels.h
+++ b/egonn_amd/csrc/kernels.h
@@ -111,9 +111,13 @@
 int dense_forward(const DenseCall& c, hipStream_t stream);
 bool dense_gate_fusable(int64_t n, int cin, int cout);
 bool dense_group3_rows(int64_t n);
-int dense_small_group3(const float* const* in, const int64_t* n, const int32_t* const* n_dev, const float* const* W, float* const* out,
-                       hipStream_t stream);
+int dense_small_group3(const float* const* in, const int64_t* n, const int32_t* const* n_dev, const float* const* W,
+                       const float* const* wfrag, float* const* out, hipStream_t stream);
 int dense_pack_frags(const float* W, int w_out_in, int cin, int cout, float* out, hipStream_t stream);
+
+constexpr int GTAIL_CIN = 128, GTAIL_MID = 192, GTAIL_OUT = 256;
+int global_tail_fused(const float* g5, int64_t ncap, const int32_t* boff, int B, const float* wf0, const float* b0, const float* wf1,
+                      const float* b1, int pow_mode, const float* p, float* partial, hipStream_t stream);
 
 int bn_fold(const float* w, const float* b, const float* rm, const float* rv, float eps, int c, float* scale,
             float* shift, hipStream_t stream);
diff --git a/egonn_amd/csrc/model.h b/egonn_amd/csrc/model.h
--- a/egonn_amd/csrc/model.h
+++ b/egonn_amd/csrc/model.h
@@ -65,7 +65,7 @@
 };
 
 struct ModelStore {
-  enum Form { RG32, RG16, SPLIT, DENSE };
+  enum Form { RG32, RG16, SPLIT, DENSE, DENSE_OI };
   struct Pack { Form form; const float* w; int K, ci, co; size_t off; const void** dst; };
   std::vector<BnRef*> bns;
   std::vector<Pack> packs;
@@ -103,6 +103,7 @@
   const float** lh_ptrs = nullptr;
   egonn::PackedKernel pk_convs[8], pk_c1[8], pk_c2[8], pk_gt[8], pk_lt[8];
   const void *pk_down[8] = {}, *pk_l1x1[8] = {};
+  const void *pk_g1x1[8] = {}, *pk_gdec[2] = {};
   egonn::MinkFpnModel* fpn = nullptr;
 };
 
@@ -124,6 +125,9 @@
 enum Pooling { POOL_GEM = 1, POOL_MAC = 2, POOL_SPOC = 3 };
 int global_pool(Pooling method, const float* x, const int32_t* boff, int B, int C, const float* p, float* partial, float* out,
                 hipStream_t st);
+bool global_tail_fusable(const MlpRef& r);
+int global_tail(const MlpRef& r, const void* const* pk, const float* g5, int64_t ncap, const int32_t* n_dev, const int32_t* boff, int B,
+                Pooling method, const float* p, bool fused, float* gh, float* gd, float* partial, float* out, hipStream_t st);
 
 bool topdown_split_supported(int C, int Cl);
 int topdown_split_forward(Ctx* ctx, int level_out, const float* x_coarse, const void* sp_tconv, const float* x_lateral,
diff --git a/egonn_amd/csrc/model.hip b/egonn_amd/csrc/model.hip
--- a/egonn_amd/csrc/model.hip
+++ b/egonn_amd/csrc/model.hip
@@ -581,6 +581,7 @@
       case RG16: EGONN_TRY(pack_rg_weights(k.w, k.K, k.ci, k.co, 1, 0, 0, out, st)); break;
       case SPLIT: EGONN_TRY(pack_split_weights(k.w, k.K, k.ci, k.co, 0, 0, out, st)); break;
       case DENSE: EGONN_TRY(dense_pack_frags(k.w, 0, k.ci, k.co, reinterpret_cast<float*>(out), st)); break;
+      case DENSE_OI: EGONN_TRY(dense_pack_frags(k.w, 1, k.ci, k.co, reinterpret_cast<float*>(out), st)); break;
     }
     *k.dst = out;
   }
@@ -620,9 +621,9 @@
   hipStream_t st = (hipStream_t)stream;
   ModelStore& S = m->store;
   S.begin();
-  auto dense = [&](const float* w, int ci, int co, const void** dst) {
+  auto dense = [&](const float* w, int ci, int co, const void** dst, ModelStore::Form form = ModelStore::DENSE) {
     *dst = nullptr;
-    if (ci % 16 == 0 && co % 16 == 0) S.add_pack(ModelStore::DENSE, w, 1, ci, co, dst);
+    if (ci % 16 == 0 && co % 16 == 0) S.add_pack(form, w, 1, ci, co, dst);
   };
   EGONN_TRY(get_tensor(m, "trunk.convs.0.kernel", {125, 1, 32}, &m->conv0));
   EGONN_TRY(get_bn(m, "trunk.bn.0", 32, &m->bn[0], &S));
@@ -641,8 +642,10 @@
     if (b.down) dense(b.down, inpl, cout, &m->pk_down[i]);
     inpl = cout;
   }
-  for (int l : {5, 6, 7})
+  for (int l : {5, 6, 7}) {
     EGONN_TRY(get_tensor(m, "global_head.conv1x1." + std::to_string(l) + ".kernel", {PLANES[l - 1], GLOBAL_CH}, &m->g1x1[l]));
+    dense(m->g1x1[l], PLANES[l - 1], GLOBAL_CH, &m->pk_g1x1[l]);
+  }
   for (int l : {6, 7}) {
     EGONN_TRY(get_tensor(m, "global_head.tconv." + std::to_string(l) + ".kernel", {8, GLOBAL_CH, GLOBAL_CH}, &m->gt[l]));
     S.add_kernel(m->gt[l], 8, GLOBAL_CH, GLOBAL_CH, true, &m->pk_gt[l]);
@@ -656,6 +659,11 @@
   m->gem_p = nullptr;
   if (m->t.count("global_pooling.pooling.p")) EGONN_TRY(get_tensor(m, "global_pooling.pooling.p", {1}, &m->gem_p));
   EGONN_TRY(get_mlp(m, "global_descriptor_decoder", GLOBAL_CH, GLOBAL_DIM + (GLOBAL_CH - GLOBAL_DIM) / 2, GLOBAL_DIM, &m->gdec));
+  m->pk_gdec[0] = m->pk_gdec[1] = nullptr;
+  if (global_tail_fusable(m->gdec)) {
+    dense(m->gdec.w0, m->gdec.cin, m->gdec.mid, &m->pk_gdec[0], ModelStore::DENSE_OI);
+    dense(m->gdec.w1, m->gdec.mid, m->gdec.cout, &m->pk_gdec[1], ModelStore::DENSE_OI);
+  }
   EGONN_TRY(get_mlp(m, "local_descriptor_decoder", LOCAL_CH, LOCAL_DIM + (LOCAL_CH - LOCAL_DIM) / 2, LOCAL_DIM, &m->ldec));
   EGONN_TRY(get_mlp(m, "local_keypoint_regressor", LOCAL_CH, LOCAL_CH / 2, 3, &m->kp));
   EGONN_TRY(get_mlp(m, "local_sigma_regressor", LOCAL_CH, LOCAL_CH / 2, 1, &m->sg));
@@ -753,15 +761,30 @@
                    .wfrag = static_cast<const float*>(wfrag), .scale = b.dn.scale, .shift = b.dn.shift, .out_bf16 = bf16};
 }
 
+static int pool_pow_mode(Pooling method) { return method == POOL_GEM ? 1 : method == POOL_MAC ? 2 : 0; }
+static int global_pool_finish(Pooling method, const float* partial, const int32_t* boff, int B, int C, const float* p, float* out,
+                              hipStream_t st) {
+  if (method == POOL_GEM) return gem_finish(partial, boff, B, C, p, out, st);
+  return pool_finish(partial, boff, B, C, pool_pow_mode(method), out, st);
+}
 int global_pool(Pooling method, const float* x, const int32_t* boff, int B, int C, const float* p, float* partial, float* out,
                 hipStream_t st) {
-  if (method == POOL_GEM) {
-    EGONN_TRY(segment_partial_sums(x, boff, B, C, 1, p, partial, st));
-    return gem_finish(partial, boff, B, C, p, out, st);
-  }
-  const int mode = method == POOL_MAC ? 2 : 0;
-  EGONN_TRY(segment_partial_sums(x, boff, B, C, mode, nullptr, partial, st));
-  return pool_finish(partial, boff, B, C, mode, out, st);
+  EGONN_TRY(segment_partial_sums(x, boff, B, C, pool_pow_mode(method), method == POOL_GEM ? p : nullptr, partial, st));
+  return global_pool_finish(method, partial, boff, B, C, p, out, st);
+}
+
+bool global_tail_fusable(const MlpRef& r) { return r.cin == GTAIL_CIN && r.mid == GTAIL_MID && r.cout == GTAIL_OUT; }
+int global_tail(const MlpRef& r, const void* const* pk, const float* g5, int64_t ncap, const int32_t* n_dev, const int32_t* boff, int B,
+                Pooling method, const float* p, bool fused, float* gh, float* gd, float* partial, float* out, hipStream_t st) {
+  if (fused) {
+    EGONN_REQUIRE(global_tail_fusable(r) && pk && pk[0] && pk[1], EGONN_ERR_STATE, "global tail: no fused form for %d->%d->%d", r.cin,
+                  r.mid, r.cout);
+    EGONN_TRY(global_tail_fused(g5, ncap, boff, B, static_cast<const float*>(pk[0]), r.b0, static_cast<const float*>(pk[1]), r.b1,
+                                pool_pow_mode(method), method == POOL_GEM ? p : nullptr, partial, st));
+    return global_pool_finish(method, partial, boff, B, r.cout, p, out, st);
+  }
+  EGONN_TRY(run_mlp(r, g5, ncap, ACT_NONE, gh, gd, st, n_dev));
+  return global_pool(method, gd, boff, B, r.cout, p, partial, out, st);
 }
 
 int block_tail(const float* x, const float* res, const int32_t* boff, int B, int64_t n, int ch, const float* eca, int eca_k,
@@ -923,7 +946,9 @@
     const int32_t* gnd[3] = {cnt + 7, cnt + 6, cnt + 5};
     const float* gw[3] = {m->g1x1[7], m->g1x1[6], m->g1x1[5]};
     float* gout[3] = {l7, l6, l5};
-    EGONN_TRY(dense_small_group3(gin, gn, gnd, gw, gout, st));
+    const float* gpk[3] = {static_cast<const float*>(m->pk_g1x1[7]), static_cast<const float*>(m->pk_g1x1[6]),
+                           static_cast<const float*>(m->pk_g1x1[5])};
+    EGONN_TRY(dense_small_group3(gin, gn, gnd, gw, switches().no_packed_laterals ? nullptr : gpk, gout, st));
     for (int lv = 6; lv >= 5; --lv) {
       ConvCall cc = conv_call(2, lv, lv == 6 ? l7 : g6f, m->pk_gt[lv + 1], GLOBAL_CH, GLOBAL_CH, 0, nullptr, 0, lv == 6 ? g6f : g5f);
       cc.residual = lv == 6 ? l6 : l5;
@@ -955,15 +980,54 @@
     }
     WALLOC(float, gh, P.cap[5] * m->gdec.mid);
     WALLOC(float, gd, P.cap[5] * GLOBAL_DIM);
-    EGONN_TRY(run_mlp(m->gdec, g5, P.cap[5], ACT_NONE, gh, gd, st, cnt + 5));
     WALLOC(float, gp, (size_t)B * SEG_CHUNKS * GLOBAL_DIM);
     const Pooling pool = (flags & EGONN_FLAG_POOL_MAC) ? POOL_MAC : (flags & EGONN_FLAG_POOL_SPOC) ? POOL_SPOC : POOL_GEM;
     EGONN_REQUIRE(pool != POOL_GEM || m->gem_p, EGONN_ERR_STATE, "forward: GeM pooling needs the tensor 'global_pooling.pooling.p'");
-    EGONN_TRY(global_pool(pool, gd, P.lv[5].boff, B, GLOBAL_DIM, m->gem_p, gp, out_global, st));
+    const bool fused_tail = !switches().no_fused_gtail && global_tail_fusable(m->gdec) && m->pk_gdec[0] && m->pk_gdec[1];
+    EGONN_TRY(global_tail(m->gdec, m->pk_gdec, g5, P.cap[5], cnt + 5, P.lv[5].boff, B, pool, m->gem_p, fused_tail, gh, gd, gp, out_global, st));
   }
 
   DBG_SYNC("global decoder + pooling");
   return EGONN_OK;
+}
+
+static size_t debug_tail_span(int64_t ncap) {
+  return align_up((size_t)ncap * GTAIL_MID * 4, 256) + align_up((size_t)ncap * GTAIL_OUT * 4, 256) +
+         align_up((size_t)GTAIL_CIN * GTAIL_MID * 4, 256) + align_up((size_t)GTAIL_MID * GTAIL_OUT * 4, 256) + 1024;
+}
+API int64_t egonn_debug_global_tail_scratch_bytes(int64_t rows_capacity) {
+  if (rows_capacity < 0 || rows_capacity >= (1ll << 31) / GTAIL_OUT) return -1;
+  return (int64_t)debug_tail_span(rows_capacity);
+}
+API int egonn_debug_global_tail(const float* g5, const int32_t* row_offsets, int batch_size, int64_t rows_capacity, const int32_t* n_dev,
+                                const float* w0, const float* b0, const float* w1, const float* b1, const float* p, int pooling, int form,
+                                float* partial, float* out, void* scratch, int64_t scratch_bytes, void* stream) {
+  EGONN_REQUIRE(g5 && row_offsets && n_dev && w0 && b0 && w1 && b1 && partial && out && scratch, EGONN_ERR_INVALID,
+                "debug_global_tail: null pointer");
+  EGONN_REQUIRE(batch_size >= 1 && batch_size <= EGONN_MAX_BATCH, EGONN_ERR_INVALID, "debug_global_tail: batch_size=%d outside [1, %d]",
+                batch_size, EGONN_MAX_BATCH);
+  EGONN_REQUIRE(rows_capacity >= 0 && rows_capacity < (1ll << 31) / GTAIL_OUT, EGONN_ERR_INVALID,
+                "debug_global_tail: rows_capacity=%lld outside [0, 2^31 / %d)", (long long)rows_capacity, GTAIL_OUT);
+  EGONN_REQUIRE(pooling >= POOL_GEM && pooling <= POOL_SPOC && (pooling != POOL_GEM || p), EGONN_ERR_INVALID,
+                "debug_global_tail: pooling=%d (1 GeM with its exponent, 2 MAC, 3 SPoC)", pooling);
+  EGONN_REQUIRE(form == 0 || form == 1, EGONN_ERR_INVALID, "debug_global_tail: form=%d (0 three launches, 1 the fused launch)", form);
+  const size_t need = debug_tail_span(rows_capacity);
+  EGONN_REQUIRE(scratch_bytes >= (int64_t)need && ((uintptr_t)scratch & 255) == 0, EGONN_ERR_INVALID,
+                "debug_global_tail: scratch needs %lld bytes, 256-byte aligned", (long long)need);
+  hipStream_t st = (hipStream_t)stream;
+  Arena ws = Arena::view(scratch, need);
+  float* gh = ws.alloc<float>((size_t)rows_capacity * GTAIL_MID);
+  float* gd = ws.alloc<float>((size_t)rows_capacity * GTAIL_OUT);
+  float* pk0 = ws.alloc<float>((size_t)GTAIL_CIN * GTAIL_MID);
+  float* pk1 = ws.alloc<float>((size_t)GTAIL_MID * GTAIL_OUT);
+  EGONN_REQUIRE(gh && gd && pk0 && pk1, EGONN_ERR_STATE, "debug_global_tail: scratch span too small");
+  const MlpRef r{.w0 = w0, .b0 = b0, .w1 = w1, .b1 = b1, .cin = GTAIL_CIN, .mid = GTAIL_MID, .cout = GTAIL_OUT};
+  const void* pk[2] = {pk0, pk1};
+  if (form == 1) {
+    EGONN_TRY(dense_pack_frags(w0, 1, r.cin, r.mid, pk0, st));
+    EGONN_TRY(dense_pack_frags(w1, 1, r.mid, r.cout, pk1, st));
+  }
+  return global_tail(r, pk, g5, rows_capacity, n_dev, row_offsets, batch_size, (Pooling)pooling, p, form == 1, gh, gd, partial, out, st);
 }
 
 API int egonn_forward_level_features(egonn_ctx* c, int level, float* out, int channels, void* stream) {
diff --git a/include/egonn_hip.h b/include/egonn_hip.h
--- a/include/egonn_hip.h
+++ b/include/egonn_hip.h
@@ -34,6 +34,12 @@
 int egonn_debug_radix_sort(uint64_t* keys_in, uint32_t* vals_in, uint64_t* keys_out, uint32_t* vals_out, int64_t n, int nbits,
                            const int64_t* n_dev, const int64_t* seg_offsets, int n_segments, int idx_bits, int either_pair,
                            int32_t* result_pair, void* scratch, int64_t scratch_bytes, void* stream);
+int egonn_debug_dense_group3(const float* const in[3], const int64_t rows_capacity[3], const int32_t* const n_dev[3],
+                             const float* const weight[3], const float* const packed[3], float* const out[3], void* stream);
+int64_t egonn_debug_global_tail_scratch_bytes(int64_t rows_capacity);
+int egonn_debug_global_tail(const float* g5, const int32_t* row_offsets, int batch_size, int64_t rows_capacity, const int32_t* n_dev,
+                            const float* w0, const float* b0, const float* w1, const float* b1, const float* p, int pooling, int form,
+                            float* partial, float* out, void* scratch, int64_t scratch_bytes, void* stream);
 
 int egonn_voxelize(egonn_ctx* ctx, const float* points, const int64_t* scan_offsets, int batch_size, int quant_mode,
                    const float* step, void* stream);
```

Measured after the change: 23380, median of 6. 2.7% higher.
